# pierrepaleo/PDWT

Measured on AMD Instinct MI355X. Metric: Mpixels/s fwd+inv DWT (4096² db4 L3), higher is better.
Workload: dtype f32; 1 GPU; 4096x4096 float32, db4, 3 levels, separable DWT fwd+inv (BASELINE.json configs[1]); levels=3, parallelism=batch-split x1 (no data-path collective)

## Files before the change

### pdwt_amd/csrc/casc_dev.hpp

```cpp
#pragma once
#include "common.hpp"

#ifndef PDWT_CASC_DIAG
#define PDWT_CASC_DIAG 0
#endif
#define CASC_DIAG_ST(row) ((PDWT_CASC_DIAG & 1) ? ((row) & 31) : (row))
#define CASC_DIAG_LD(row) ((PDWT_CASC_DIAG & 2) ? ((row) & 31) : (row))

namespace pdwt {

template <int HLEN>
struct CascGeom {
    static constexpr int C = HLEN / 2 - 1;
    static constexpr int NB1 = C > 0 ? (C + 3) / 4 : 0;
    static constexpr int NB2 = C > 0 ? (C + 1) / 2 : 0;
    static constexpr int NBT = NB1 + NB2;
    static constexpr int WIN1 = 4 * (2 * NB1 + 1);
    static constexpr int WIN2 = 2 * (2 * NB2 + 1);
    static constexpr int MAXVL = 64 - 2 * NBT;
};

struct CascMap {
    int cpx;
    int strips;
    int gy;
    int flags;
    const void* tbl;
};
__host__ __device__ inline int casc_chunk_start(int g, int strip, int units, int gy, int strips, int cpx, int d)
{
    if (g >= gy) return units;
    int b = (int)(((long long)g * units) / gy);
    if (d != 0) {
        int bal = 0;
        for (int q = 0; q < g; q++) bal += (((q * strips + strip) / cpx) & 1) ? -1 : 1;
        b += d * bal;
    }
    return b;
}

struct CascBands {
    float *H1, *V1, *D1, *A2, *H2, *V2, *D2;
};
struct CascBatchF {
    const float* in;
    CascBands b;
};

template <int HLEN>
struct CascInvGeom {
    static constexpr int H2 = HLEN / 2;
    static constexpr int C = H2 / 2;
    static constexpr int SHIFT = (H2 & 1) ? 0 : 1;
    static constexpr int NB1 = C > 0 ? (C + 1) / 2 : 0;
    static constexpr int NB2 = C;
    static constexpr int NBT = NB1 + NB2;
    static constexpr int WIN1 = 2 * (2 * NB1 + 1);
    static constexpr int WIN2 = 2 * NB2 + 1;
    static constexpr int MAXVL = 64 - 2 * NBT;
    static constexpr int BASE = (C - SHIFT) & 1;
    static constexpr int VM_SB = H2 * (4 + 2 * (3 + 2));
};
struct CascInvBands {
    const float *A2, *H2, *V2, *D2, *H1, *V1, *D1;
};
struct CascInv3B {
    const float *A3, *H3, *V3, *D3;
};
struct CascBatchI {
    CascInvBands b;
    CascInv3B b3;
    float* out;
};


constexpr size_t kCascTraceOff = 1u << 20;
#ifdef PDWT_CASC_TRACE
#define CASC_TRACE_DECL unsigned long long casc_tr_[8] = {0, 0, 0, 0, 0, 0, 0, 0}
#define CASC_TRACE(i) casc_tr_[i] = wall_clock64()
#define CASC_TRACE_STORE(trash, wave_id, aux)                                                             \
    do {                                                                                                   \
        if ((threadIdx.x & 63) == 0) {                                                                     \
            unsigned long long* p_ = reinterpret_cast<unsigned long long*>((trash) + kCascTraceOff) + (size_t)(wave_id) * 8; \
            for (int i_ = 0; i_ < 7; i_++) p_[i_] = casc_tr_[i_];                                          \
            p_[7] = (unsigned long long)(aux);                                                             \
        }                                                                                                  \
    } while (0)
#else
#define CASC_TRACE_DECL
#define CASC_TRACE(i)
#define CASC_TRACE_STORE(trash, wave_id, aux)
#endif

int inv2d_casc3_f32(const float* A2, const float* H2, const float* V2, const float* D2, const float* H1, const float* V1, const float* D1,
                    const float* A3, const float* H3, const float* V3, const float* D3, float* out, float* trash, int nr, int nc, int hlen,
                    const Taps2<float>& f, const CascBatchI* d_tbl = nullptr, int nimg = 1);

int inv2d_cascw_f32(const float* A2, const float* H2, const float* V2, const float* D2, const float* H1, const float* V1, const float* D1,
                    const float* A3, const float* H3, const float* V3, const float* D3, float* out, float* trash, int nr, int nc, int hlen,
                    const Taps2<float>& f);

}
```

### pdwt_amd/csrc/common.hpp

```cpp
#pragma once
#include <atomic>
#include <hip/hip_runtime.h>
#include <hip/hip_ext.h>
#include <stddef.h>
#include <stdint.h>

#include "../../include/pdwt_hip.h"

namespace pdwt {

void set_last_error(hipError_t e, const char* what, const char* file, int line);

#define PDWT_HIP_TRY(expr)                                              \
    do {                                                                \
        hipError_t _e = (expr);                                         \
        if (_e != hipSuccess) {                                         \
            ::pdwt::set_last_error(_e, #expr, __FILE__, __LINE__);      \
            return PDWT_EHIP;                                           \
        }                                                               \
    } while (0)

hipStream_t stream();

enum KernelId {
    K_FWD2D_FUSED = 0,
    K_INV2D_FUSED,
    K_ANA_ROWS,
    K_ANA_COLS,
    K_SYN_COLS,
    K_SYN_ROWS,
    K_SWT_ANA_ROWS,
    K_SWT_ANA_COLS,
    K_SWT_SYN_COLS,
    K_SWT_SYN_ROWS,
    K_HAAR2D_FWD,
    K_HAAR2D_INV,
    K_HAAR1D_FWD,
    K_HAAR1D_INV,
    K_SOFT_THRESH,
    K_ABS_SUM,
    K_ABS_SUM_FINAL,
    K_FWD2D_CASC,
    K_INV2D_CASC,
    K_FWD2D_STREAM,
    K_INV2D_STREAM,
    K_FWD2D_SMALL,
    K_INV2D_SMALL,
    K_FWD2D_F64,
    K_INV2D_F64,
    K_THRESH_SUM,
    K_COUNT
};

struct KTimer {
    int id;
    hipEvent_t e0 = nullptr, e1 = nullptr;
    bool ext = false;
    explicit KTimer(int kernel_id, bool attach_to_launch = false);
    ~KTimer();
};
#define PDWT_LAUNCH_KT(kt, kernel, grid, block, lds, ...)                                                                  \
    do {                                                                                                                   \
        if ((kt).e0 && (kt).e1) hipExtLaunchKernelGGL(kernel, grid, block, lds, pdwt::stream(), (kt).e0, (kt).e1, 0, __VA_ARGS__); \
        else hipLaunchKernelGGL(kernel, grid, block, lds, pdwt::stream(), __VA_ARGS__);                                    \
    } while (0)

template <auto Kernel>
inline int lds_opt_in()
{
    static std::atomic<unsigned long long> done{0};
    int dev = 0;
    PDWT_HIP_TRY(hipGetDevice(&dev));
    const unsigned long long bit = 1ull << (dev & 63);
    if (!(done.load(std::memory_order_relaxed) & bit)) {
        PDWT_HIP_TRY(hipFuncSetAttribute((const void*)Kernel, hipFuncAttributeMaxDynamicSharedMemorySize, 160 * 1024));
        done.fetch_or(bit, std::memory_order_relaxed);
    }
    return PDWT_OK;
}

int lds_opt_in_ptr(const void* kernel);

unsigned long long* clock_probe_slot(int slot);
inline int clock_probe_size_class(int rows) { int c = 0; while ((rows << c) < 16384 && c < 7) c++; return c; }
constexpr int kClockProbeAllBlocks = 16384;
unsigned long long* clock_probe_all(int* all);
__device__ __forceinline__ void clock_probe_stamp(unsigned long long* probe, int second, int all = 0)
{
    if (probe && (all || (blockIdx.x == 0 && blockIdx.y == 0))) {
        unsigned long long* const p = probe + (all ? 4 * (size_t)blockIdx.x : (size_t)0);
        const unsigned long long c = clock64(), t = wall_clock64();
        if (threadIdx.x == 0) {
            p[2 * second] = c;
            p[2 * second + 1] = t;
        }
    }
}

enum KnobId {
    KN_FORCE_TWOPASS = 0,
    KN_TILED_COLS,
    KN_CASC,
    KN_CASC_WAVES,
    KN_CASC_NV,
    KN_CASC_MIN,
    KN_CASC_IWAVES,
    KN_CASC_IPFD,
    KN_CASC_WG,
    KN_CASC_IWG,
    KN_CASC_L3,
    KN_CASC_SPEC,
    KN_CASC_XCDW,
    KN_DWT1D_LDS_KB,
    KN_STREAM,
    KN_STREAM_R,
    KN_STREAM_WAVES,
    KN_STREAM_NARROW,
    KN_SMALL,
    KN_ROWS_TR,
    KN_RING_R,
    KN_RING_WAVES,
    KN_SWTF,
    KN_SWTF_M,
    KN_SWTF_MI,
    KN_SWTF_XCD,
    KN_SWTF_ALT,
    KN_SWTF_PERM,
    KN_SWTF_F64,
    KN_F64_LDS,
    KN_F64_LDS_MIN,
    KN_F64_LDS_WGS,
    KN_F64_LDS_MINGROUPS,
    KN_F64_LDS_SKEW,
    KN_NORM2SQ_REF1D,
    KN_NORM_IN_THRESHOLD,
    KN_SELFCHECK,
    KN_DWT1D_F64,
    KN_SWTF_LONG,
    KN_F64_TAIL,
    KN_EXP0,
    KN_EXP1,
    KN_EXP2,
    KN_EXP3,
    KN_NONSEP_TILED,
    KN_F64_LAT,
    KN_F64_LAT_MIN,
    KN_DWT1D_NT_MB,
    KN_COUNT
};
int knob(KnobId id);
bool counted_waits_ok();
void stat_casc_spec(int inverse);
int knob_set(const char* name, int value);
int knob_get(const char* name, int* value);

__host__ __device__ inline int div2(int n) { return (n + 1) >> 1; }
inline int idiv_up(int a, int b) { return (a + b - 1) / b; }

__device__ __forceinline__ int wrap_ext(int s, int n)
{
    const int np = n + (n & 1);
    if ((unsigned)s >= (unsigned)np) {
        s %= np;
        if (s < 0) s += np;
    }
    return (s == n) ? n - 1 : s;
}
__device__ __forceinline__ int wrap_per(int s, int n)
{
    if ((unsigned)s >= (unsigned)n) {
        s %= n;
        if (s < 0) s += n;
    }
    return s;
}

template <typename T>
struct Taps2 {
    T a[PDWT_MAX_FILTER_WIDTH];
    T b[PDWT_MAX_FILTER_WIDTH];
};

template <typename T> struct FiltersOf;
template <> struct FiltersOf<float> { using type = pdwt_filters_f32; };
template <> struct FiltersOf<double> { using type = pdwt_filters_f64; };

template <typename T>
inline Taps2<T> taps_fwd(const typename FiltersOf<T>::type* f)
{
    Taps2<T> t;
    for (int i = 0; i < PDWT_MAX_FILTER_WIDTH; i++) { t.a[i] = f->L[i]; t.b[i] = f->H[i]; }
    return t;
}
template <typename T>
inline Taps2<T> taps_inv(const typename FiltersOf<T>::type* f, T scale = T(1))
{
    Taps2<T> t;
    for (int i = 0; i < PDWT_MAX_FILTER_WIDTH; i++) { t.a[i] = f->IL[i] * scale; t.b[i] = f->IH[i] * scale; }
    return t;
}

template <typename T> __device__ __forceinline__ T fma_t(T a, T b, T c);
template <> __device__ __forceinline__ float fma_t<float>(float a, float b, float c) { return __builtin_fmaf(a, b, c); }
template <> __device__ __forceinline__ double fma_t<double>(double a, double b, double c) { return __builtin_fma(a, b, c); }

struct BandGeom {
    int nbands;
    int Nr[3 * 32 + 1], Nc[3 * 32 + 1];
    size_t alloc_elems[3 * 32 + 1];
};
int band_geometry(const pdwt_info& w, BandGeom* g);

}
```

### pdwt_amd/csrc/dwt.hip

```cpp
#include <stdlib.h>
#include <string.h>

#include "common.hpp"
#include "cols_ring.hpp"
#include "rows_tr.hpp"
#include "dwt1d_fused.hpp"
#include <new>
#include <vector>

#include "dwt_lds.hpp"
#include "dwt_lat.hpp"
#include "dwt_stream.hpp"
#include "dwt_casc.hpp"
#include "casc_dev.hpp"

namespace pdwt {

constexpr int kThreads = 256;

template <typename T, int HLEN, int TX, int TY>
__global__ __launch_bounds__(kThreads) void k_fwd2d_fused(const T* __restrict__ in, T* __restrict__ cA, T* __restrict__ cH,
                                                           T* __restrict__ cV, T* __restrict__ cD, int Nr, int Nc, int hlen_rt,
                                                           Taps2<T> f)
{
    extern __shared__ __attribute__((aligned(16))) unsigned char smem[];
    const int hlen = HLEN > 0 ? HLEN : hlen_rt;
    const int c = (hlen & 1) ? hlen / 2 : hlen / 2 - 1;
    const int RIN = 2 * TY + hlen - 2;
    const int CIN = 2 * TX + hlen - 2;
    const int CINP = CIN | 1;
    T* s_in = reinterpret_cast<T*>(smem);
    T* s_lo = s_in + RIN * CINP;
    T* s_hi = s_lo + RIN * TX;

    const int Nr2 = div2(Nr), Nc2 = div2(Nc);
    const int x0 = blockIdx.x * TX, y0 = blockIdx.y * TY;
    const int xb = 2 * x0 - c, yb = 2 * y0 - c;
    const int tx = threadIdx.x & 63, ty = threadIdx.x >> 6;

    const bool interior = (xb >= 0) && (xb + CIN <= Nc) && (yb >= 0) && (yb + RIN <= Nr);
    if (interior) {
        for (int r = ty; r < RIN; r += 4) {
            const T* row = in + (size_t)(yb + r) * Nc + xb;
            for (int cc = tx; cc < CIN; cc += 64) s_in[r * CINP + cc] = row[cc];
        }
    } else {
        for (int r = ty; r < RIN; r += 4) {
            const T* row = in + (size_t)wrap_ext(yb + r, Nr) * Nc;
            for (int cc = tx; cc < CIN; cc += 64) s_in[r * CINP + cc] = row[wrap_ext(xb + cc, Nc)];
        }
    }
    __syncthreads();

    for (int r = ty; r < RIN; r += 4) {
        const T* p = s_in + r * CINP + 2 * tx;
        T lo = 0, hi = 0;
#pragma unroll
        for (int j = 0; j < hlen; j++) {
            const T v = p[j];
            lo = fma_t(v, f.a[hlen - 1 - j], lo);
            hi = fma_t(v, f.b[hlen - 1 - j], hi);
        }
        s_lo[r * TX + tx] = lo;
        s_hi[r * TX + tx] = hi;
    }
    __syncthreads();

    const int gx = x0 + tx;
    for (int y = ty; y < TY; y += 4) {
        T a = 0, h = 0, v = 0, d = 0;
        const T* pl = s_lo + (2 * y) * TX + tx;
        const T* ph = s_hi + (2 * y) * TX + tx;
#pragma unroll
        for (int j = 0; j < hlen; j++) {
            const T l = pl[j * TX], g = ph[j * TX];
            const T fl = f.a[hlen - 1 - j], fh = f.b[hlen - 1 - j];
            a = fma_t(l, fl, a);
            h = fma_t(l, fh, h);
            v = fma_t(g, fl, v);
            d = fma_t(g, fh, d);
        }
        const int gy = y0 + y;
        if (gy < Nr2 && gx < Nc2) {
            const size_t o = (size_t)gy * Nc2 + gx;
            cA[o] = a;
            cH[o] = h;
            cV[o] = v;
            cD[o] = d;
        }
    }
}

template <typename T, int HLEN, int TX, int TY>
__global__ __launch_bounds__(kThreads) void k_inv2d_fused(const T* __restrict__ cA, const T* __restrict__ cH, const T* __restrict__ cV,
                                                           const T* __restrict__ cD, T* __restrict__ out, int Nri, int Nci, int Nro,
                                                           int Nco, int hlen_rt, Taps2<T> f)
{
    extern __shared__ __attribute__((aligned(16))) unsigned char smem[];
    const int hlen = HLEN > 0 ? HLEN : hlen_rt;
    const int h2 = hlen / 2;
    const int c = h2 / 2;
    const int shift = (h2 & 1) ? 0 : 1;
    const int RC = TY + h2;
    const int CC = TX + h2;
    const int CCP = CC | 1;
    T* s_A = reinterpret_cast<T*>(smem);
    T* s_H = s_A + RC * CCP;
    T* s_V = s_H + RC * CCP;
    T* s_D = s_V + RC * CCP;
    T* s_t1 = s_D + RC * CCP;
    T* s_t2 = s_t1 + 2 * TY * CCP;

    const int x0 = blockIdx.x * TX, y0 = blockIdx.y * TY;
    const int xb = x0 - c, yb = y0 - c;
    const int tx = threadIdx.x & 63, ty = threadIdx.x >> 6;

    const bool interior = (xb >= 0) && (xb + CC <= Nci) && (yb >= 0) && (yb + RC <= Nri);
    for (int r = ty; r < RC; r += 4) {
        const size_t ro = (size_t)(interior ? yb + r : wrap_per(yb + r, Nri)) * Nci;
        for (int cc = tx; cc < CC; cc += 64) {
            const size_t o = ro + (interior ? xb + cc : wrap_per(xb + cc, Nci));
            const int s = r * CCP + cc;
            s_A[s] = cA[o];
            s_H[s] = cH[o];
            s_V[s] = cV[o];
            s_D[s] = cD[o];
        }
    }
    __syncthreads();

    for (int gyl = ty; gyl < 2 * TY; gyl += 4) {
        const int gp = gyl + shift;
        const int pl = gp >> 1, off = 1 - (gp & 1);
        for (int cc = tx; cc < CC; cc += 64) {
            T sa = 0, sh = 0, sv = 0, sd = 0;
            const int base = pl * CCP + cc;
#pragma unroll
            for (int j = 0; j < h2; j++) {
                const int k = hlen - 1 - (2 * j + off);
                const T fl = f.a[k], fh = f.b[k];
                const int s = base + j * CCP;
                sa = fma_t(s_A[s], fl, sa);
                sh = fma_t(s_H[s], fh, sh);
                sv = fma_t(s_V[s], fl, sv);
                sd = fma_t(s_D[s], fh, sd);
            }
            s_t1[gyl * CCP + cc] = sa + sh;
            s_t2[gyl * CCP + cc] = sv + sd;
        }
    }
    __syncthreads();

    for (int gyl = ty; gyl < 2 * TY; gyl += 4) {
        const int gy = 2 * y0 + gyl;
        if (gy >= Nro) break;
        for (int u = tx; u < TX; u += 64) {
            T res[2];
#pragma unroll
            for (int e = 0; e < 2; e++) {
                const int gp = 2 * u + e + shift;
                const int pl = gp >> 1, off = 1 - ((e + shift) & 1);
                T s1 = 0, s2 = 0;
                const int base = gyl * CCP + pl;
#pragma unroll
                for (int j = 0; j < h2; j++) {
                    const int k = hlen - 1 - (2 * j + off);
                    s1 = fma_t(s_t1[base + j], f.a[k], s1);
                    s2 = fma_t(s_t2[base + j], f.b[k], s2);
                }
                res[e] = s1 + s2;
            }
            const int gx = 2 * x0 + 2 * u;
            if (gx < Nco) out[(size_t)gy * Nco + gx] = res[0];
            if (gx + 1 < Nco) out[(size_t)gy * Nco + gx + 1] = res[1];
        }
    }
}

template <typename T, int HLEN, int TXO>
__global__ __launch_bounds__(kThreads) void k_ana_rows(const T* __restrict__ in, T* __restrict__ lo, T* __restrict__ hi, int Nr, int Nc,
                                                        int hlen_rt, Taps2<T> f)
{
    extern __shared__ __attribute__((aligned(16))) unsigned char smem[];
    const int hlen = HLEN > 0 ? HLEN : hlen_rt;
    const int c = (hlen & 1) ? hlen / 2 : hlen / 2 - 1;
    const int CIN = 2 * TXO + hlen - 2;
    const int CINP = CIN | 1;
    const int lane = threadIdx.x & 63, w = threadIdx.x >> 6;
    T* s = reinterpret_cast<T*>(smem) + w * CINP;
    const int Nc2 = div2(Nc);
    const int x0 = blockIdx.x * TXO;
    const int xb = 2 * x0 - c;
    const int row = blockIdx.y * 4 + w;
    if (row < Nr) {
        const T* src = in + (size_t)row * Nc;
        if (xb >= 0 && xb + CIN <= Nc) {
            for (int cc = lane; cc < CIN; cc += 64) s[cc] = src[xb + cc];
        } else {
            for (int cc = lane; cc < CIN; cc += 64) s[cc] = src[wrap_ext(xb + cc, Nc)];
        }
    }
    __syncthreads();
    if (row >= Nr) return;
    for (int i = lane; i < TXO; i += 64) {
        const int gx = x0 + i;
        if (gx >= Nc2) break;
        const T* p = s + 2 * i;
        T l = 0, h = 0;
#pragma unroll
        for (int j = 0; j < hlen; j++) {
            const T v = p[j];
            l = fma_t(v, f.a[hlen - 1 - j], l);
            h = fma_t(v, f.b[hlen - 1 - j], h);
        }
        lo[(size_t)row * Nc2 + gx] = l;
        hi[(size_t)row * Nc2 + gx] = h;
    }
}

template <typename T, int HLEN, int TYO>
__global__ __launch_bounds__(kThreads) void k_ana_cols(const T* __restrict__ t1, const T* __restrict__ t2, T* __restrict__ cA,
                                                        T* __restrict__ cH, T* __restrict__ cV, T* __restrict__ cD, int Nr, int Ncw,
                                                        int hlen_rt, Taps2<T> f)
{
    extern __shared__ __attribute__((aligned(16))) unsigned char smem[];
    const int hlen = HLEN > 0 ? HLEN : hlen_rt;
    const int c = (hlen & 1) ? hlen / 2 : hlen / 2 - 1;
    const int RIN = 2 * TYO + hlen - 2;
    T* s1 = reinterpret_cast<T*>(smem);
    T* s2 = s1 + RIN * 64;
    const int tx = threadIdx.x & 63, ty = threadIdx.x >> 6;
    const int Nr2 = div2(Nr);
    const int gx = blockIdx.x * 64 + tx;
    const int y0 = blockIdx.y * TYO;
    const int yb = 2 * y0 - c;
    if (gx < Ncw) {
        for (int r = ty; r < RIN; r += 4) {
            const size_t o = (size_t)wrap_ext(yb + r, Nr) * Ncw + gx;
            s1[r * 64 + tx] = t1[o];
            s2[r * 64 + tx] = t2[o];
        }
    }
    __syncthreads();
    if (gx >= Ncw) return;
    for (int y = ty; y < TYO; y += 4) {
        const int gy = y0 + y;
        if (gy >= Nr2) break;
        T a = 0, h = 0, v = 0, d = 0;
        const T* p1 = s1 + (2 * y) * 64 + tx;
        const T* p2 = s2 + (2 * y) * 64 + tx;
#pragma unroll
        for (int j = 0; j < hlen; j++) {
            const T l = p1[j * 64], g = p2[j * 64];
            const T fl = f.a[hlen - 1 - j], fh = f.b[hlen - 1 - j];
            a = fma_t(l, fl, a);
            h = fma_t(l, fh, h);
            v = fma_t(g, fl, v);
            d = fma_t(g, fh, d);
        }
        const size_t o = (size_t)gy * Ncw + gx;
        cA[o] = a;
        cH[o] = h;
        cV[o] = v;
        cD[o] = d;
    }
}

template <typename T, int HLEN, int TYC>
__global__ __launch_bounds__(kThreads) void k_syn_cols(const T* __restrict__ cA, const T* __restrict__ cH, const T* __restrict__ cV,
                                                        const T* __restrict__ cD, T* __restrict__ t1, T* __restrict__ t2, int Nri,
                                                        int Nc, int Nro, int hlen_rt, Taps2<T> f)
{
    extern __shared__ __attribute__((aligned(16))) unsigned char smem[];
    const int hlen = HLEN > 0 ? HLEN : hlen_rt;
    const int h2 = hlen / 2;
    const int c = h2 / 2;
    const int shift = (h2 & 1) ? 0 : 1;
    const int RC = TYC + h2;
    T* s_A = reinterpret_cast<T*>(smem);
    T* s_H = s_A + RC * 64;
    T* s_V = s_H + RC * 64;
    T* s_D = s_V + RC * 64;
    const int tx = threadIdx.x & 63, ty = threadIdx.x >> 6;
    const int gx = blockIdx.x * 64 + tx;
    const int y0 = blockIdx.y * TYC;
    const int yb = y0 - c;
    if (gx < Nc) {
        for (int r = ty; r < RC; r += 4) {
            const size_t o = (size_t)wrap_per(yb + r, Nri) * Nc + gx;
            const int s = r * 64 + tx;
            s_A[s] = cA[o];
            s_H[s] = cH[o];
            s_V[s] = cV[o];
            s_D[s] = cD[o];
        }
    }
    __syncthreads();
    if (gx >= Nc) return;
    for (int gyl = ty; gyl < 2 * TYC; gyl += 4) {
        const int gy = 2 * y0 + gyl;
        if (gy >= Nro) break;
        const int gp = gyl + shift;
        const int pl = gp >> 1, off = 1 - (gp & 1);
        T sa = 0, sh = 0, sv = 0, sd = 0;
        const int base = pl * 64 + tx;
#pragma unroll
        for (int j = 0; j < h2; j++) {
            const int k = hlen - 1 - (2 * j + off);
            const T fl = f.a[k], fh = f.b[k];
            const int s = base + j * 64;
            sa = fma_t(s_A[s], fl, sa);
            sh = fma_t(s_H[s], fh, sh);
            sv = fma_t(s_V[s], fl, sv);
            sd = fma_t(s_D[s], fh, sd);
        }
        t1[(size_t)gy * Nc + gx] = sa + sh;
        t2[(size_t)gy * Nc + gx] = sv + sd;
    }
}

template <typename T, int HLEN, int TXC>
__global__ __launch_bounds__(kThreads) void k_syn_rows(const T* __restrict__ a, const T* __restrict__ d, T* __restrict__ out, int Nr,
                                                        int Nci, int Nco, int hlen_rt, Taps2<T> f)
{
    extern __shared__ __attribute__((aligned(16))) unsigned char smem[];
    const int hlen = HLEN > 0 ? HLEN : hlen_rt;
    const int h2 = hlen / 2;
    const int c = h2 / 2;
    const int shift = (h2 & 1) ? 0 : 1;
    const int CC = TXC + h2;
    const int lane = threadIdx.x & 63, w = threadIdx.x >> 6;
    T* sa = reinterpret_cast<T*>(smem) + w * 2 * CC;
    T* sd = sa + CC;
    const int x0 = blockIdx.x * TXC;
    const int xb = x0 - c;
    const int row = blockIdx.y * 4 + w;
    if (row < Nr) {
        const T* pa = a + (size_t)row * Nci;
        const T* pd = d + (size_t)row * Nci;
        for (int cc = lane; cc < CC; cc += 64) {
            const int sx = wrap_per(xb + cc, Nci);
            sa[cc] = pa[sx];
            sd[cc] = pd[sx];
        }
    }
    __syncthreads();
    if (row >= Nr) return;
    for (int u = lane; u < TXC; u += 64) {
        const int gx = 2 * x0 + 2 * u;
        if (gx >= Nco) break;
        T res[2];
#pragma unroll
        for (int e = 0; e < 2; e++) {
            const int gp = 2 * u + e + shift;
            const int pl = gp >> 1, off = 1 - ((e + shift) & 1);
            T s1 = 0, s2 = 0;
#pragma unroll
            for (int j = 0; j < h2; j++) {
                const int k = hlen - 1 - (2 * j + off);
                s1 = fma_t(sa[pl + j], f.a[k], s1);
                s2 = fma_t(sd[pl + j], f.b[k], s2);
            }
            res[e] = s1 + s2;
        }
        out[(size_t)row * Nco + gx] = res[0];
        if (gx + 1 < Nco) out[(size_t)row * Nco + gx + 1] = res[1];
    }
}

template <typename K>
static int set_lds(K kernel, size_t bytes)
{
    if (bytes > 64 * 1024) return lds_opt_in_ptr((const void*)kernel);
    return PDWT_OK;
}

static bool force_twopass() { return knob(KN_FORCE_TWOPASS) == 1; }
static bool tiled_cols_forced() { return knob(KN_TILED_COLS) == 1; }

constexpr int FTX = 64, FTY = 16;
constexpr size_t kFusedLdsBudget = 64 * 1024;

template <typename T>
static size_t fwd_fused_lds(int hlen)
{
    const int RIN = 2 * FTY + hlen - 2, CINP = (2 * FTX + hlen - 2) | 1;
    return ((size_t)RIN * CINP + 2 * (size_t)RIN * FTX) * sizeof(T);
}
template <typename T>
static size_t inv_fused_lds(int hlen)
{
    const int h2 = hlen / 2, RC = FTY + h2, CCP = (FTX + h2) | 1;
    return (4 * (size_t)RC * CCP + 2 * (size_t)(2 * FTY) * CCP) * sizeof(T);
}

#define PDWT_CHECK_LAUNCH() PDWT_HIP_TRY(hipGetLastError())

#define PDWT_TILED_HLENS(X) X(4) X(6) X(8) X(10) X(12) X(14) X(16) X(18) X(20) X(24) X(30) X(40)

template <typename T>
static int launch_ana_rows(const T* in, T* lo, T* hi, int Nr, int Nc, int hlen, const Taps2<T>& f)
{
    if constexpr (sizeof(T) == 8) {
        const int rc = ana_rows_tr_f64(in, lo, hi, Nr, Nc, hlen, f);
        if (rc <= 0) return rc;
    }
    constexpr int TXO = 256;
    const size_t lds = 4 * (size_t)((2 * TXO + hlen - 2) | 1) * sizeof(T);
    dim3 grid(idiv_up(div2(Nc), TXO), idiv_up(Nr, 4));
    void (*k)(const T*, T*, T*, int, int, int, Taps2<T>);
    switch (hlen) {
#define X(H) case H: k = k_ana_rows<T, H, TXO>; break;
        PDWT_TILED_HLENS(X)
#undef X
        default: k = k_ana_rows<T, 0, TXO>; break;
    }
    KTimer kt(K_ANA_ROWS);
    hipLaunchKernelGGL(k, grid, dim3(kThreads), lds, stream(), in, lo, hi, Nr, Nc, hlen, f);
    PDWT_CHECK_LAUNCH();
    return PDWT_OK;
}

template <typename T>
static int launch_syn_rows(const T* a, const T* d, T* out, int Nr, int Nci, int Nco, int hlen, const Taps2<T>& f)
{
    if constexpr (sizeof(T) == 8) {
        const int rc = syn_rows_tr_f64(a, d, out, Nr, Nci, Nco, hlen, f);
        if (rc <= 0) return rc;
    }
    constexpr int TXC = 128;
    const size_t lds = 4 * 2 * (size_t)(TXC + hlen / 2) * sizeof(T);
    dim3 grid(idiv_up(Nci, TXC), idiv_up(Nr, 4));
    void (*k)(const T*, const T*, T*, int, int, int, int, Taps2<T>);
    switch (hlen) {
#define X(H) case H: k = k_syn_rows<T, H, TXC>; break;
        PDWT_TILED_HLENS(X)
#undef X
        default: k = k_syn_rows<T, 0, TXC>; break;
    }
    KTimer kt(K_SYN_ROWS);
    hipLaunchKernelGGL(k, grid, dim3(kThreads), lds, stream(), a, d, out, Nr, Nci, Nco, hlen, f);
    PDWT_CHECK_LAUNCH();
    return PDWT_OK;
}

template <typename T>
static int launch_ana_cols(const T* t1, const T* t2, T* cA, T* cH, T* cV, T* cD, int Nr, int Ncw, int hlen, const Taps2<T>& f)
{
    if (!tiled_cols_forced()) {
        KTimer kt(K_ANA_COLS);
        const int rc = ana_cols_ring<T>(t1, cA, cH, Nr, Ncw, hlen, f, t2, cV, cD);
        if (rc <= 0) return rc;
    }
    constexpr int TYO = 16;
    const size_t lds = 2 * (size_t)(2 * TYO + hlen - 2) * 64 * sizeof(T);
    void (*k)(const T*, const T*, T*, T*, T*, T*, int, int, int, Taps2<T>);
    switch (hlen) {
#define X(H) case H: k = k_ana_cols<T, H, TYO>; break;
        PDWT_TILED_HLENS(X)
#undef X
        default: k = k_ana_cols<T, 0, TYO>; break;
    }
    if (set_lds(k, lds) != PDWT_OK) return PDWT_EHIP;
    dim3 grid(idiv_up(Ncw, 64), idiv_up(div2(Nr), TYO));
    KTimer kt(K_ANA_COLS);
    hipLaunchKernelGGL(k, grid, dim3(kThreads), lds, stream(), t1, t2, cA, cH, cV, cD, Nr, Ncw, hlen, f);
    PDWT_CHECK_LAUNCH();
    return PDWT_OK;
}

template <typename T>
static int launch_syn_cols(const T* cA, const T* cH, const T* cV, const T* cD, T* t1, T* t2, int Nri, int Nc, int Nro, int hlen,
                           const Taps2<T>& f)
{
    if (!tiled_cols_forced()) {
        KTimer kt(K_SYN_COLS);
        const int rc = syn_cols_ring<T>(cA, cH, t1, Nri, Nc, Nro, hlen, f, cV, cD, t2);
        if (rc <= 0) return rc;
    }
    constexpr int TYC = 16;
    const size_t lds = 4 * (size_t)(TYC + hlen / 2) * 64 * sizeof(T);
    void (*k)(const T*, const T*, const T*, const T*, T*, T*, int, int, int, int, Taps2<T>);
    switch (hlen) {
#define X(H) case H: k = k_syn_cols<T, H, TYC>; break;
        PDWT_TILED_HLENS(X)
#undef X
        default: k = k_syn_cols<T, 0, TYC>; break;
    }
    if (set_lds(k, lds) != PDWT_OK) return PDWT_EHIP;
    dim3 grid(idiv_up(Nc, 64), idiv_up(Nri, TYC));
    KTimer kt(K_SYN_COLS);
    hipLaunchKernelGGL(k, grid, dim3(kThreads), lds, stream(), cA, cH, cV, cD, t1, t2, Nri, Nc, Nro, hlen, f);
    PDWT_CHECK_LAUNCH();
    return PDWT_OK;
}

template <typename T>
static int level_fwd2d(const T* in, T* cA, T* cH, T* cV, T* cD, T* t1, T* t2, size_t trash_floats, int nr, int nc, int hlen, const Taps2<T>& f,
                       T* taps_dev)
{
    if constexpr (sizeof(T) == 8) {
        if (!force_twopass()) {
            int rc = fwd2d_f64_lat(in, cA, cH, cV, cD, nr, nc, hlen, f);
            if (rc <= 0) return rc;
            rc = fwd2d_f64_lds(in, cA, cH, cV, cD, taps_dev, nr, nc, hlen, f);
            if (rc <= 0) return rc;
        }
    }
    if constexpr (sizeof(T) == 4) {
        if (!force_twopass()) {
            int rc = fwd2d_stream_f32(in, cA, cH, cV, cD, (float*)t1, trash_floats, nr, nc, hlen, f);
            if (rc <= 0) return rc;
            rc = fwd2d_f32_lds(in, cA, cH, cV, cD, nr, nc, hlen, f);
            if (rc <= 0) return rc;
        }
    }
    const size_t lds = fwd_fused_lds<T>(hlen);
    if (lds <= kFusedLdsBudget && !force_twopass()) {
        dim3 grid(idiv_up(div2(nc), FTX), idiv_up(div2(nr), FTY));
        void (*k)(const T*, T*, T*, T*, T*, int, int, int, Taps2<T>);
        switch (hlen) {
#define X(H) case H: k = k_fwd2d_fused<T, H, FTX, FTY>; break;
            PDWT_TILED_HLENS(X)
#undef X
            default: k = k_fwd2d_fused<T, 0, FTX, FTY>; break;
        }
        KTimer kt(K_FWD2D_FUSED);
        hipLaunchKernelGGL(k, grid, dim3(kThreads), lds, stream(), in, cA, cH, cV, cD, nr, nc, hlen, f);
        PDWT_CHECK_LAUNCH();
        return PDWT_OK;
    }
    int rc = launch_ana_rows(in, t1, t2, nr, nc, hlen, f);
    if (rc != PDWT_OK) return rc;
    return launch_ana_cols(t1, t2, cA, cH, cV, cD, nr, div2(nc), hlen, f);
}

template <typename T>
static int level_inv2d(const T* cA, const T* cH, const T* cV, const T* cD, T* out, T* t1, T* t2, int nri, int nci, int nro, int nco,
                       int hlen, const Taps2<T>& f, T* taps_dev)
{
    if constexpr (sizeof(T) == 8) {
        if (!force_twopass()) {
            int rc = inv2d_f64_lat(cA, cH, cV, cD, out, nri, nci, nro, nco, hlen, f);
            if (rc <= 0) return rc;
            rc = inv2d_f64_lds(cA, cH, cV, cD, out, taps_dev, nri, nci, nro, nco, hlen, f);
            if (rc <= 0) return rc;
        }
    }
    if constexpr (sizeof(T) == 4) {
        if (!force_twopass()) {
            int rc = inv2d_stream_f32(cA, cH, cV, cD, out, nri, nci, nro, nco, hlen, f);
            if (rc <= 0) return rc;
            rc = inv2d_f32_lds(cA, cH, cV, cD, out, nri, nci, nro, nco, hlen, f);
            if (rc <= 0) return rc;
        }
    }
    const size_t lds = inv_fused_lds<T>(hlen);
    if (lds <= kFusedLdsBudget && !force_twopass()) {
        dim3 grid(idiv_up(nci, FTX), idiv_up(nri, FTY));
        void (*k)(const T*, const T*, const T*, const T*, T*, int, int, int, int, int, Taps2<T>);
        switch (hlen) {
#define X(H) case H: k = k_inv2d_fused<T, H, FTX, FTY>; break;
            PDWT_TILED_HLENS(X)
#undef X
            default: k = k_inv2d_fused<T, 0, FTX, FTY>; break;
        }
        KTimer kt(K_INV2D_FUSED);
        hipLaunchKernelGGL(k, grid, dim3(kThreads), lds, stream(), cA, cH, cV, cD, out, nri, nci, nro, nco, hlen, f);
        PDWT_CHECK_LAUNCH();
        return PDWT_OK;
    }
    int rc = launch_syn_cols(cA, cH, cV, cD, t1, t2, nri, nci, nro, hlen, f);
    if (rc != PDWT_OK) return rc;
    return launch_syn_rows(t1, t2, out, nro, nci, nco, hlen, f);
}

template <typename T>
struct Scratch {
    T *t1, *t2, *ping[2];
    size_t trash_floats;
    bool t1_is_trash;
    Scratch(T* tmp, int Nr, int Nc, int ndims)
    {
        t1_is_trash = (ndims == 2) && ((size_t)Nr * div2(Nc) * sizeof(T) >= kStreamTrashFloats * sizeof(float)) && Nr >= 32;
        auto up = [](size_t n) { return (n + 63) & ~(size_t)63; };
        const size_t half = up((size_t)Nr * div2(Nc));
        trash_floats = (ndims == 2) ? 2 * half * sizeof(T) / sizeof(float) : 0;
        const size_t quarter = up((size_t)(ndims == 2 ? div2(Nr) : Nr) * div2(Nc));
        t1 = tmp;
        t2 = t1 + half;
        if (ndims == 2) {
            ping[0] = t2 + half;
            ping[1] = ping[0] + quarter;
        } else {
            ping[0] = tmp;
            ping[1] = tmp + quarter;
        }
    }
};

static int check_args(const void* img, const void* coeffs, const void* tmp, const pdwt_info& w, int ndims, bool need_filters, const void* f,
                      int fhlen)
{
    if (!img || !coeffs || !tmp) return PDWT_EINVAL;
    if (w.Nr < 1 || w.Nc < 1 || w.nlevels < 1 || w.nlevels > 32) return PDWT_EINVAL;
    if (w.ndims != ndims) return PDWT_EINVAL;
    if (need_filters) {
        if (!f) return PDWT_EINVAL;
        if (w.hlen < 2 || w.hlen > PDWT_MAX_FILTER_WIDTH || fhlen != w.hlen) return PDWT_EINVAL;
    }
    return PDWT_OK;
}

template <typename T>
static int forward_separable(T* d_image, T** c, T* d_tmp, pdwt_info w, const typename FiltersOf<T>::type* filt)
{
    int rc = check_args(d_image, c, d_tmp, w, 2, true, filt, filt ? filt->hlen : 0);
    if (rc != PDWT_OK) return rc;
    const Taps2<T> f = taps_fwd<T>(filt);
    Scratch<T> s(d_tmp, w.Nr, w.Nc, 2);
    const T* in = d_image;
    int nr = w.Nr, nc = w.Nc;
    int pp = 0;
    for (int lev = 0; lev < w.nlevels; lev++) {
        if constexpr (sizeof(T) == 4) {
            if (lev + 1 < w.nlevels && !force_twopass()) {
                T* a2 = (lev + 2 == w.nlevels) ? c[0] : s.ping[pp];
                float* trash = s.t1_is_trash ? (float*)s.t1 : nullptr;
                rc = fwd2d_casc_f32(in, c[3 * lev + 1], c[3 * lev + 2], c[3 * lev + 3], a2, c[3 * lev + 4], c[3 * lev + 5], c[3 * lev + 6],
                                    trash, nr, nc, w.hlen, f);
                if (rc < 0) return rc;
                if (rc == PDWT_OK) {
                    in = a2;
                    pp ^= 1;
                    nr = div2(div2(nr));
                    nc = div2(div2(nc));
                    lev++;
                    continue;
                }
            }
        }
        T* aout = (lev == w.nlevels - 1) ? c[0] : s.ping[pp];
        rc = level_fwd2d(in, aout, c[3 * lev + 1], c[3 * lev + 2], c[3 * lev + 3], s.t1, s.t2, s.trash_floats, nr, nc, w.hlen, f,
                         d_tmp + pdwt_tmp_elems(w) - 256);
        if (rc != PDWT_OK) return rc;
        in = aout;
        pp ^= 1;
        nr = div2(nr);
        nc = div2(nc);
    }
    return PDWT_OK;
}

template <typename T>
static int inverse_separable(T* d_image, T** c, T* d_tmp, pdwt_info w, const typename FiltersOf<T>::type* filt)
{
    int rc = check_args(d_image, c, d_tmp, w, 2, true, filt, filt ? filt->hlen : 0);
    if (rc != PDWT_OK) return rc;
    const Taps2<T> f = taps_inv<T>(filt);
    Scratch<T> s(d_tmp, w.Nr, w.Nc, 2);
    int tNr[34], tNc[34];
    tNr[0] = w.Nr;
    tNc[0] = w.Nc;
    for (int i = 1; i <= w.nlevels; i++) {
        tNr[i] = div2(tNr[i - 1]);
        tNc[i] = div2(tNc[i - 1]);
    }
    const T* a = c[0];
    int top = w.nlevels - 1;
    int pp = (a == s.ping[0]) ? 1 : 0;
    for (int i = top; i >= 0; i--) {
        if constexpr (sizeof(T) == 4) {
            float* trash = s.t1_is_trash ? (float*)s.t1 : nullptr;
            if (i >= 2 && !(i & 1) && !force_twopass()) {
                T* out = (i == 2) ? d_image : s.ping[pp];
                rc = inv2d_cascw_f32(nullptr, c[3 * i - 2], c[3 * i - 1], c[3 * i], c[3 * i - 5], c[3 * i - 4], c[3 * i - 3], a, c[3 * i + 1],
                                     c[3 * i + 2], c[3 * i + 3], out, trash, tNr[i - 2], tNc[i - 2], w.hlen, f);
                if (rc < 0) return rc;
                if (rc == PDWT_OK) {
                    a = out;
                    pp ^= 1;
                    i -= 2;
                    continue;
                }
            }
            if ((i & 1) && !force_twopass()) {
                T* out = (i == 1) ? d_image : s.ping[pp];
                rc = inv2d_cascw_f32(a, c[3 * i + 1], c[3 * i + 2], c[3 * i + 3], c[3 * i - 2], c[3 * i - 1], c[3 * i], nullptr, nullptr, nullptr,
                                     nullptr, out, trash, tNr[i - 1], tNc[i - 1], w.hlen, f);
                if (rc < 0) return rc;
                if (rc == PDWT_OK) {
                    a = out;
                    pp ^= 1;
                    i--;
                    continue;
                }
                rc = inv2d_casc_f32(a, c[3 * i + 1], c[3 * i + 2], c[3 * i + 3], c[3 * i - 2], c[3 * i - 1], c[3 * i], out, trash, tNr[i - 1],
                                    tNc[i - 1], w.hlen, f);
                if (rc < 0) return rc;
                if (rc == PDWT_OK) {
                    a = out;
                    pp ^= 1;
                    i--;
                    continue;
                }
            }
        }
        T* out = (i == 0) ? d_image : s.ping[pp];
        rc = level_inv2d(a, c[3 * i + 1], c[3 * i + 2], c[3 * i + 3], out, s.t1, s.t2, tNr[i + 1], tNc[i + 1], tNr[i], tNc[i], w.hlen, f,
                         d_tmp + pdwt_tmp_elems(w) - 256);
        if (rc != PDWT_OK) return rc;
        a = out;
        pp ^= 1;
    }
    return PDWT_OK;
}

template <typename T>
static int forward_separable_1d(T* d_image, T** c, T* d_tmp, pdwt_info w, const typename FiltersOf<T>::type* filt)
{
    int rc = check_args(d_image, c, d_tmp, w, 1, true, filt, filt ? filt->hlen : 0);
    if (rc != PDWT_OK) return rc;
    const Taps2<T> f = taps_fwd<T>(filt);
    if (!force_twopass()) {
        rc = fwd1d_fused<T>(d_image, c, w, f);
        if (rc <= 0) return rc;
    }
    Scratch<T> s(d_tmp, w.Nr, w.Nc, 1);
    const T* in = d_image;
    int nc = w.Nc;
    for (int lev = 0; lev < w.nlevels; lev++) {
        T* aout = (lev == w.nlevels - 1) ? c[0] : s.ping[lev & 1];
        rc = launch_ana_rows(in, aout, c[lev + 1], w.Nr, nc, w.hlen, f);
        if (rc != PDWT_OK) return rc;
        in = aout;
        nc = div2(nc);
    }
    return PDWT_OK;
}

template <typename T>
static int inverse_separable_1d(T* d_image, T** c, T* d_tmp, pdwt_info w, const typename FiltersOf<T>::type* filt)
{
    int rc = check_args(d_image, c, d_tmp, w, 1, true, filt, filt ? filt->hlen : 0);
    if (rc != PDWT_OK) return rc;
    const Taps2<T> f = taps_inv<T>(filt);
    if (!force_twopass()) {
        rc = inv1d_fused<T>(d_image, c, w, f);
        if (rc <= 0) return rc;
    }
    Scratch<T> s(d_tmp, w.Nr, w.Nc, 1);
    int tNc[34];
    tNc[0] = w.Nc;
    for (int i = 1; i <= w.nlevels; i++) tNc[i] = div2(tNc[i - 1]);
    const T* a = c[0];
    for (int i = w.nlevels - 1; i >= 0; i--) {
        T* out = (i == 0) ? d_image : s.ping[i & 1];
        rc = launch_syn_rows(a, (const T*)c[i + 1], out, w.Nr, tNc[i + 1], tNc[i], w.hlen, f);
        if (rc != PDWT_OK) return rc;
        a = out;
    }
    return PDWT_OK;
}


static inline bool b2_al16(const void* p) { return ((uintptr_t)p & 15) == 0; }
template <typename T> void* haar_batch_create(int nimg, T* const* d_images, T** const* d_coeffs, T* const* d_tmps, pdwt_info w);
template <typename T> int haar_batch_forward(void* batch);
template <typename T> int haar_batch_inverse(void* batch);
template <typename T> void haar_batch_destroy(void* batch);
void* swt_batch_create_f32(int nimg, float* const* d_images, float** const* d_coeffs, float* const* d_tmps, pdwt_info w);
int swt_batch_forward_f32(void* batch, const pdwt_filters_f32* filt);
int swt_batch_inverse_f32(void* batch, const pdwt_filters_f32* filt);
void swt_batch_destroy_f32(void* batch);
struct BatchHaar {
    int kind, dev, elem;
    void* hb;
};
static void* batch_swt_create(int nimg, float* const* d_images, float** const* d_coeffs, float* const* d_tmps, pdwt_info w)
{
    BatchHaar* B = new (std::nothrow) BatchHaar();
    if (!B) return nullptr;
    B->kind = 3;
    B->elem = 4;
    B->hb = (hipGetDevice(&B->dev) == hipSuccess) ? swt_batch_create_f32(nimg, d_images, d_coeffs, d_tmps, w) : nullptr;
    if (!B->hb) {
        delete B;
        return nullptr;
    }
    return B;
}
template <typename T>
static void* batch_haar_create(int nimg, T* const* d_images, T** const* d_coeffs, T* const* d_tmps, pdwt_info w)
{
    BatchHaar* B = new (std::nothrow) BatchHaar();
    if (!B) return nullptr;
    B->kind = 2;
    B->elem = (int)sizeof(T);
    B->hb = (hipGetDevice(&B->dev) == hipSuccess) ? haar_batch_create<T>(nimg, d_images, d_coeffs, d_tmps, w) : nullptr;
    if (!B->hb) {
        delete B;
        return nullptr;
    }
    return B;
}
struct Batch2D {
    int kind;
    int nimg, dev;
    pdwt_info w;
    size_t trash_floats;
    int lev_nr[33], lev_nc[33];
    StreamBatchF* d_fwd;
    StreamBatchI* d_inv;
    CascBatchF* d_cf;
    CascBatchI* d_ci;
    CascBatchF cf0;
    CascBatchI ci0;
    float* trash0;
};

static Batch2D* batch2d_create(int nimg, float* const* d_images, float** const* d_coeffs, float* const* d_tmps, pdwt_info w, int hlen)
{
    if (nimg < 1 || nimg > 65535 || !d_images || !d_coeffs || !d_tmps || w.ndims != 2 || w.do_swt || w.nlevels < 1 || w.nlevels > 32) return nullptr;
    if (force_twopass()) return nullptr;
    int nr = w.Nr, nc = w.Nc;
    for (int lev = 0; lev < w.nlevels; lev++) {
        if (!fwd2d_stream_takes(nr, nc, hlen) || !inv2d_stream_takes(nr / 2, nc / 2, hlen)) return nullptr;
        nr /= 2;
        nc /= 2;
    }
    Scratch<float> probe(d_tmps[0], w.Nr, w.Nc, 2);
    if (probe.trash_floats < 1024) return nullptr;
    Batch2D* B = new (std::nothrow) Batch2D();
    if (!B) return nullptr;
    B->kind = 0;
    B->nimg = nimg;
    B->w = w;
    B->trash_floats = probe.trash_floats;
    B->d_fwd = nullptr;
    B->d_inv = nullptr;
    B->d_cf = nullptr;
    B->d_ci = nullptr;
    B->trash0 = nullptr;
    if (hipGetDevice(&B->dev) != hipSuccess) {
        delete B;
        return nullptr;
    }
    const int L = w.nlevels;
    std::vector<StreamBatchF> hf((size_t)L * nimg);
    std::vector<StreamBatchI> hi((size_t)L * nimg);
    for (int b = 0; b < nimg; b++) {
        float* const* c = d_coeffs[b];
        Scratch<float> s(d_tmps[b], w.Nr, w.Nc, 2);
        if (!d_images[b] || !c || !d_tmps[b] || !b2_al16(d_images[b])) {
            delete B;
            return nullptr;
        }
        const float* in = d_images[b];
        int pp = 0;
        for (int lev = 0; lev < L; lev++) {
            float* aout = (lev == L - 1) ? c[0] : s.ping[pp];
            hf[(size_t)lev * nimg + b] = StreamBatchF{in, aout, c[3 * lev + 1], c[3 * lev + 2], c[3 * lev + 3], (float*)s.t1};
            if (!b2_al16(aout) || !b2_al16(c[3 * lev + 1]) || !b2_al16(c[3 * lev + 2]) || !b2_al16(c[3 * lev + 3])) {
                delete B;
                return nullptr;
            }
            in = aout;
            pp ^= 1;
        }
        const float* a = c[0];
        pp = 0;
        for (int i = L - 1; i >= 0; i--) {
            float* out = (i == 0) ? d_images[b] : s.ping[pp];
            hi[(size_t)i * nimg + b] = StreamBatchI{a, c[3 * i + 1], c[3 * i + 2], c[3 * i + 3], out};
            a = out;
            pp ^= 1;
        }
    }
    nr = w.Nr;
    nc = w.Nc;
    for (int lev = 0; lev <= L; lev++) {
        B->lev_nr[lev] = nr;
        B->lev_nc[lev] = nc;
        nr /= 2;
        nc /= 2;
    }
    const size_t bf = hf.size() * sizeof(StreamBatchF), bi = hi.size() * sizeof(StreamBatchI);
    B->d_fwd = (StreamBatchF*)pdwt_malloc(bf);
    B->d_inv = (StreamBatchI*)pdwt_malloc(bi);
    bool ok = B->d_fwd && B->d_inv && pdwt_memcpy_h2d(B->d_fwd, hf.data(), bf) == PDWT_OK && pdwt_memcpy_h2d(B->d_inv, hi.data(), bi) == PDWT_OK;
    if (ok && L >= 2) {
        std::vector<CascBatchF> hcf((size_t)nimg);
        std::vector<CascBatchI> hci((size_t)nimg);
        for (int b = 0; b < nimg; b++) {
            float* const* c = d_coeffs[b];
            hcf[b] = CascBatchF{d_images[b], CascBands{c[1], c[2], c[3], hf[(size_t)1 * nimg + b].cA, c[4], c[5], c[6]}};
            hci[b].b = CascInvBands{L == 2 ? hi[(size_t)1 * nimg + b].cA : nullptr, c[4], c[5], c[6], c[1], c[2], c[3]};
            hci[b].b3 = (L >= 3) ? CascInv3B{hi[(size_t)2 * nimg + b].cA, c[7], c[8], c[9]} : CascInv3B{nullptr, nullptr, nullptr, nullptr};
            hci[b].out = d_images[b];
        }
        B->cf0 = hcf[0];
        B->ci0 = hci[0];
        Scratch<float> s0(d_tmps[0], w.Nr, w.Nc, 2);
        B->trash0 = s0.t1_is_trash ? (float*)s0.t1 : nullptr;
        const size_t cf = hcf.size() * sizeof(CascBatchF), ci = hci.size() * sizeof(CascBatchI);
        B->d_cf = (CascBatchF*)pdwt_malloc(cf);
        B->d_ci = (CascBatchI*)pdwt_malloc(ci);
        ok = B->d_cf && B->d_ci && pdwt_memcpy_h2d(B->d_cf, hcf.data(), cf) == PDWT_OK && pdwt_memcpy_h2d(B->d_ci, hci.data(), ci) == PDWT_OK;
    }
    if (!ok) {
        pdwt_free(B->d_fwd);
        pdwt_free(B->d_inv);
        pdwt_free(B->d_cf);
        pdwt_free(B->d_ci);
        delete B;
        return nullptr;
    }
    return B;
}

struct Batch2DDev {
    int prev = -1;
    bool switched = false;
    explicit Batch2DDev(int dev)
    {
        if (hipGetDevice(&prev) == hipSuccess && prev != dev) switched = (hipSetDevice(dev) == hipSuccess);
    }
    ~Batch2DDev()
    {
        if (switched) (void)hipSetDevice(prev);
    }
};

static int batch2d_forward(Batch2D* B, const pdwt_filters_f32* filt)
{
    if (!B || !filt || filt->hlen != B->w.hlen) return PDWT_EINVAL;
    Batch2DDev on_dev(B->dev);
    const Taps2<float> f = taps_fwd<float>(filt);
    int lev0 = 0;
    if (B->d_cf && B->trash0) {
        const CascBands& b = B->cf0.b;
        const int rc = fwd2d_casc_f32(B->cf0.in, b.H1, b.V1, b.D1, b.A2, b.H2, b.V2, b.D2, B->trash0, B->lev_nr[0], B->lev_nc[0], B->w.hlen, f,
                                      B->d_cf, B->nimg);
        if (rc < 0) return rc;
        if (rc == PDWT_OK) lev0 = 2;
    }
    for (int lev = lev0; lev < B->w.nlevels; lev++) {
        const int rc = fwd2d_stream_batch_f32(B->d_fwd + (size_t)lev * B->nimg, B->nimg, B->trash_floats, B->lev_nr[lev], B->lev_nc[lev], B->w.hlen, f);
        if (rc != PDWT_OK) return rc < 0 ? rc : PDWT_EINVAL;
    }
    return PDWT_OK;
}

static int batch2d_inverse(Batch2D* B, const pdwt_filters_f32* filt)
{
    if (!B || !filt || filt->hlen != B->w.hlen) return PDWT_EINVAL;
    Batch2DDev on_dev(B->dev);
    const Taps2<float> f = taps_inv<float>(filt);
    const int L = B->w.nlevels;
    const int ncasc = (L >= 3) ? 3 : 2;
    bool casc = B->d_ci && B->trash0 && L >= 2 && knob(KN_CASC) == 1 && knob(KN_CASC_IWG) != 1 && knob(KN_CASC_L3) == 1 && stream_enabled() &&
                !((long long)knob(KN_CASC_MIN) > (long long)B->lev_nr[0] * B->lev_nc[0]);
    int next = L - 1;
    for (; next >= (casc ? ncasc : 0); next--) {
        const int rc = inv2d_stream_batch_f32(B->d_inv + (size_t)next * B->nimg, B->nimg, B->lev_nr[next + 1], B->lev_nc[next + 1], B->w.hlen, f);
        if (rc != PDWT_OK) return rc < 0 ? rc : PDWT_EINVAL;
    }
    if (casc) {
        const CascInvBands& b = B->ci0.b;
        const CascInv3B& b3 = B->ci0.b3;
        const int rc = inv2d_casc3_f32(b.A2, b.H2, b.V2, b.D2, b.H1, b.V1, b.D1, b3.A3, b3.H3, b3.V3, b3.D3, B->ci0.out, B->trash0, B->lev_nr[0],
                                       B->lev_nc[0], B->w.hlen, f, B->d_ci, B->nimg);
        if (rc < 0) return rc;
        if (rc == PDWT_OK) return PDWT_OK;
    }
    for (; next >= 0; next--) {
        const int rc = inv2d_stream_batch_f32(B->d_inv + (size_t)next * B->nimg, B->nimg, B->lev_nr[next + 1], B->lev_nc[next + 1], B->w.hlen, f);
        if (rc != PDWT_OK) return rc < 0 ? rc : PDWT_EINVAL;
    }
    return PDWT_OK;
}

struct Batch2D64 {
    int kind;
    int nimg, dev;
    pdwt_info w;
    int lev_nr[34], lev_nc[34];
    unsigned long long* d_fwd;
    unsigned long long* d_inv;
};

static Batch2D64* batch2d_create_f64(int nimg, double* const* d_images, double** const* d_coeffs, double* const* d_tmps, pdwt_info w)
{
    if (nimg < 1 || nimg > 65535 || !d_images || !d_coeffs || !d_tmps || w.ndims != 2 || w.do_swt || w.nlevels < 1 || w.nlevels > 32) return nullptr;
    if (force_twopass() || w.hlen < 2 || w.hlen > 40 || (w.hlen & 1) || knob(KN_F64_LDS) < 1) return nullptr;
    Batch2D64* B = new (std::nothrow) Batch2D64();
    if (!B) return nullptr;
    B->kind = 1;
    B->nimg = nimg;
    B->w = w;
    B->d_fwd = B->d_inv = nullptr;
    if (hipGetDevice(&B->dev) != hipSuccess) {
        delete B;
        return nullptr;
    }
    const int L = w.nlevels;
    int nr = w.Nr, nc = w.Nc;
    for (int lev = 0; lev <= L; lev++) {
        B->lev_nr[lev] = nr;
        B->lev_nc[lev] = nc;
        const int hp = ((w.hlen + 7) / 8) * 8;
        if (lev < L && (nr < 16 || nr < hp || nc < hp || div2(nr) < hp || div2(nc) < 2)) {
            delete B;
            return nullptr;
        }
        nr = div2(nr);
        nc = div2(nc);
    }
    std::vector<unsigned long long> hf((size_t)L * nimg * 5), hi((size_t)L * nimg * 5);
    for (int b = 0; b < nimg; b++) {
        double* const* c = d_coeffs[b];
        if (!d_images[b] || !c || !d_tmps[b]) {
            delete B;
            return nullptr;
        }
        Scratch<double> sc(d_tmps[b], w.Nr, w.Nc, 2);
        const double* in = d_images[b];
        int pp = 0;
        for (int lev = 0; lev < L; lev++) {
            double* aout = (lev == L - 1) ? c[0] : sc.ping[pp];
            unsigned long long* e = &hf[((size_t)lev * nimg + b) * 5];
            e[0] = (unsigned long long)(uintptr_t)in;
            e[1] = (unsigned long long)(uintptr_t)aout;
            e[2] = (unsigned long long)(uintptr_t)c[3 * lev + 1];
            e[3] = (unsigned long long)(uintptr_t)c[3 * lev + 2];
            e[4] = (unsigned long long)(uintptr_t)c[3 * lev + 3];
            if (!aout || !c[3 * lev + 1] || !c[3 * lev + 2] || !c[3 * lev + 3]) {
                delete B;
                return nullptr;
            }
            in = aout;
            pp ^= 1;
        }
        const double* a = c[0];
        pp = 0;
        for (int i = L - 1; i >= 0; i--) {
            double* out = (i == 0) ? d_images[b] : sc.ping[pp];
            unsigned long long* e = &hi[((size_t)i * nimg + b) * 5];
            e[0] = (unsigned long long)(uintptr_t)a;
            e[1] = (unsigned long long)(uintptr_t)c[3 * i + 1];
            e[2] = (unsigned long long)(uintptr_t)c[3 * i + 2];
            e[3] = (unsigned long long)(uintptr_t)c[3 * i + 3];
            e[4] = (unsigned long long)(uintptr_t)out;
            a = out;
            pp ^= 1;
        }
    }
    const size_t bytes = hf.size() * sizeof(unsigned long long);
    B->d_fwd = (unsigned long long*)pdwt_malloc(bytes);
    B->d_inv = (unsigned long long*)pdwt_malloc(bytes);
    if (!B->d_fwd || !B->d_inv || pdwt_memcpy_h2d(B->d_fwd, hf.data(), bytes) != PDWT_OK || pdwt_memcpy_h2d(B->d_inv, hi.data(), bytes) != PDWT_OK) {
        pdwt_free(B->d_fwd);
        pdwt_free(B->d_inv);
        delete B;
        return nullptr;
    }
    return B;
}

static int batch2d_forward_f64(Batch2D64* B, const pdwt_filters_f64* filt)
{
    if (!B || !filt || filt->hlen != B->w.hlen) return PDWT_EINVAL;
    Batch2DDev on_dev(B->dev);
    const Taps2<double> f = taps_fwd<double>(filt);
    for (int lev = 0; lev < B->w.nlevels; lev++) {
        const int rc = fwd2d_f64_lds_batch(B->d_fwd + (size_t)lev * B->nimg * 5, B->nimg, B->lev_nr[lev], B->lev_nc[lev], B->w.hlen, f);
        if (rc != PDWT_OK) return rc < 0 ? rc : PDWT_EINVAL;
    }
    return PDWT_OK;
}
static int batch2d_inverse_f64(Batch2D64* B, const pdwt_filters_f64* filt)
{
    if (!B || !filt || filt->hlen != B->w.hlen) return PDWT_EINVAL;
    Batch2DDev on_dev(B->dev);
    const Taps2<double> f = taps_inv<double>(filt);
    for (int i = B->w.nlevels - 1; i >= 0; i--) {
        const int rc = inv2d_f64_lds_batch(B->d_inv + (size_t)i * B->nimg * 5, B->nimg, B->lev_nr[i + 1], B->lev_nc[i + 1], B->lev_nr[i], B->lev_nc[i], B->w.hlen, f);
        if (rc != PDWT_OK) return rc < 0 ? rc : PDWT_EINVAL;
    }
    return PDWT_OK;
}

}

template <typename F>
static bool bank_is_haar(const F* f)
{
    if (!f || f->hlen != 2) return false;
    const double r = 0.70710678118654752440, tol = 1e-6;
    auto near = [&](double a, double b) { return a - b <= tol && b - a <= tol; };
    return near(f->L[0], r) && near(f->L[1], r) && near(f->H[0], -r) && near(f->H[1], r) && near(f->IL[0], r) && near(f->IL[1], r) && near(f->IH[0], r) && near(f->IH[1], -r);
}

using namespace pdwt;

extern "C" {
static bool batch_is_haar(const pdwt_info& w) { return w.hlen == 2 && w.ndims == 2 && !w.do_swt; }
void* pdwt_batch2d_create_f64(int nimg, double* const* d_images, double** const* d_coeffs, double* const* d_tmps, pdwt_info info)
{
    if (batch_is_haar(info)) return batch_haar_create<double>(nimg, d_images, d_coeffs, d_tmps, info);
    return batch2d_create_f64(nimg, d_images, d_coeffs, d_tmps, info);
}
static int batch_kind(const void* batch, int elem)
{
    if (!batch) return -1;
    const int k = *(const int*)batch;
    if (k == 0 || k == 3) return elem == 4 ? k : -1;
    if (k == 1) return elem == 8 ? k : -1;
    if (k == 2) return ((const BatchHaar*)batch)->elem == elem ? k : -1;
    return -1;
}
int pdwt_batch2d_forward_f64(void* batch, const pdwt_filters_f64* f)
{
    const int k = batch_kind(batch, 8);
    if (k == 2) {
        if (!bank_is_haar(f)) return PDWT_EINVAL;
        Batch2DDev on_dev(((BatchHaar*)batch)->dev);
        return haar_batch_forward<double>(((BatchHaar*)batch)->hb);
    }
    return k == 1 ? batch2d_forward_f64((Batch2D64*)batch, f) : PDWT_EINVAL;
}
int pdwt_batch2d_inverse_f64(void* batch, const pdwt_filters_f64* f)
{
    const int k = batch_kind(batch, 8);
    if (k == 2) {
        if (!bank_is_haar(f)) return PDWT_EINVAL;
        Batch2DDev on_dev(((BatchHaar*)batch)->dev);
        return haar_batch_inverse<double>(((BatchHaar*)batch)->hb);
    }
    return k == 1 ? batch2d_inverse_f64((Batch2D64*)batch, f) : PDWT_EINVAL;
}
void* pdwt_batch2d_create_f32(int nimg, float* const* d_images, float** const* d_coeffs, float* const* d_tmps, pdwt_info info)
{
    if (batch_is_haar(info)) return batch_haar_create<float>(nimg, d_images, d_coeffs, d_tmps, info);
    if (info.do_swt) return batch_swt_create(nimg, d_images, d_coeffs, d_tmps, info);
    return batch2d_create(nimg, d_images, d_coeffs, d_tmps, info, info.hlen);
}
int pdwt_batch2d_forward_f32(void* batch, const pdwt_filters_f32* f)
{
    const int k = batch_kind(batch, 4);
    if (k == 2 || k == 3) {
        if (k == 2 && !bank_is_haar(f)) return PDWT_EINVAL;
        Batch2DDev on_dev(((BatchHaar*)batch)->dev);
        return k == 2 ? haar_batch_forward<float>(((BatchHaar*)batch)->hb) : swt_batch_forward_f32(((BatchHaar*)batch)->hb, f);
    }
    return k == 0 ? batch2d_forward((Batch2D*)batch, f) : PDWT_EINVAL;
}
int pdwt_batch2d_inverse_f32(void* batch, const pdwt_filters_f32* f)
{
    const int k = batch_kind(batch, 4);
    if (k == 2 || k == 3) {
        if (k == 2 && !bank_is_haar(f)) return PDWT_EINVAL;
        Batch2DDev on_dev(((BatchHaar*)batch)->dev);
        return k == 2 ? haar_batch_inverse<float>(((BatchHaar*)batch)->hb) : swt_batch_inverse_f32(((BatchHaar*)batch)->hb, f);
    }
    return k == 0 ? batch2d_inverse((Batch2D*)batch, f) : PDWT_EINVAL;
}
void pdwt_batch2d_destroy(void* batch)
{
    if (!batch) return;
    const int k = *(const int*)batch;
    if (k == 2 || k == 3) {
        BatchHaar* H = (BatchHaar*)batch;
        if (k == 3)
            swt_batch_destroy_f32(H->hb);
        else if (H->elem == 8)
            haar_batch_destroy<double>(H->hb);
        else
            haar_batch_destroy<float>(H->hb);
        delete H;
    } else if (k == 1) {
        Batch2D64* B = (Batch2D64*)batch;
        pdwt_free(B->d_fwd);
        pdwt_free(B->d_inv);
        delete B;
    } else if (k == 0) {
        Batch2D* B = (Batch2D*)batch;
        pdwt_free(B->d_fwd);
        pdwt_free(B->d_inv);
        pdwt_free(B->d_cf);
        pdwt_free(B->d_ci);
        delete B;
    }
}
void pdwt_batch2d_destroy_f64(void* batch) { pdwt_batch2d_destroy(batch); }
int pdwt_debug_set(const char* key, int value) { return pdwt::knob_set(key, value); }
int pdwt_debug_get(const char* key, int* value) { return pdwt::knob_get(key, value); }
size_t pdwt_tmp_elems(pdwt_info w) { return 2 * (size_t)(w.Nr > 0 ? w.Nr : 0) * (size_t)(w.Nc > 0 ? w.Nc : 0) + 1024; }
int pdwt_forward_separable_f32(float* i, float** c, float* t, pdwt_info w, const pdwt_filters_f32* f) { return forward_separable<float>(i, c, t, w, f); }
int pdwt_forward_separable_f64(double* i, double** c, double* t, pdwt_info w, const pdwt_filters_f64* f) { return forward_separable<double>(i, c, t, w, f); }
int pdwt_inverse_separable_f32(float* i, float** c, float* t, pdwt_info w, const pdwt_filters_f32* f) { return inverse_separable<float>(i, c, t, w, f); }
int pdwt_inverse_separable_f64(double* i, double** c, double* t, pdwt_info w, const pdwt_filters_f64* f) { return inverse_separable<double>(i, c, t, w, f); }
int pdwt_forward_separable_1d_f32(float* i, float** c, float* t, pdwt_info w, const pdwt_filters_f32* f) { return forward_separable_1d<float>(i, c, t, w, f); }
int pdwt_forward_separable_1d_f64(double* i, double** c, double* t, pdwt_info w, const pdwt_filters_f64* f) { return forward_separable_1d<double>(i, c, t, w, f); }
int pdwt_inverse_separable_1d_f32(float* i, float** c, float* t, pdwt_info w, const pdwt_filters_f32* f) { return inverse_separable_1d<float>(i, c, t, w, f); }
int pdwt_inverse_separable_1d_f64(double* i, double** c, double* t, pdwt_info w, const pdwt_filters_f64* f) { return inverse_separable_1d<double>(i, c, t, w, f); }
}
```

### pdwt_amd/csrc/dwt_casc.hip

```cpp
#include "dwt_casc.hpp"

#include <algorithm>

#include "dwt_stream.hpp"
#include "stream_dev.hpp"
#include "casc_dev.hpp"

namespace pdwt {

constexpr int casc_fwd_stores(int p) { return 3 + 4 * (p & 1); }
template <int DIST>
constexpr int casc_fwd_after(int p)
{
    int n = casc_fwd_stores(p);
    for (int k = 1; k < DIST; k++) n += 2 + casc_fwd_stores(p + k);
    return n;
}

template <int HLEN>
constexpr int casc_fwd_region_bytes() { return (HLEN - 2) * 64 * (16 + 8); }

#define PDWT_VB_F0 " op_sel_hi:[0,1,0]"
#define PDWT_VB_N0 " op_sel_hi:[0,1,1]"
#define PDWT_VB_F1 " op_sel:[1,0,0] op_sel_hi:[1,1,0]"
#define PDWT_VB_N1 " op_sel:[1,0,0]"
template <bool WITH_VD>
__device__ __forceinline__ void col_pass8x2(v2f& ah0, v2f& ah1, v2f& vd0, v2f& vd1, v2f a0, v2f a1, v2f a2, v2f a3, v2f a4, v2f a5, v2f a6, v2f a7, v2f b0, v2f b1,
                                            v2f b2, v2f b3, v2f b4, v2f b5, v2f b6, v2f b7, v2f t0, v2f t1, v2f t2, v2f t3, v2f t4, v2f t5, v2f t6, v2f t7)
{
#define PDWT_CP_ROW(A, B, T, AC)                                                                                              \
    "v_pk_fma_f32 %0, " A ", " T ", " AC "0\n\tv_pk_fma_f32 %1, " B ", " T ", " AC "1\n\t"
    if constexpr (WITH_VD) {
        asm("v_pk_fma_f32 %0, %4, %20, 0" PDWT_VB_F0 "\n\tv_pk_fma_f32 %1, %12, %20, 0" PDWT_VB_F0 "\n\tv_pk_fma_f32 %2, %4, %20, 0" PDWT_VB_F1 "\n\tv_pk_fma_f32 %3, %12, %20, 0" PDWT_VB_F1
            "\n\tv_pk_fma_f32 %0, %5, %21, %0" PDWT_VB_N0 "\n\tv_pk_fma_f32 %1, %13, %21, %1" PDWT_VB_N0 "\n\tv_pk_fma_f32 %2, %5, %21, %2" PDWT_VB_N1 "\n\tv_pk_fma_f32 %3, %13, %21, %3" PDWT_VB_N1
            "\n\tv_pk_fma_f32 %0, %6, %22, %0" PDWT_VB_N0 "\n\tv_pk_fma_f32 %1, %14, %22, %1" PDWT_VB_N0 "\n\tv_pk_fma_f32 %2, %6, %22, %2" PDWT_VB_N1 "\n\tv_pk_fma_f32 %3, %14, %22, %3" PDWT_VB_N1
            "\n\tv_pk_fma_f32 %0, %7, %23, %0" PDWT_VB_N0 "\n\tv_pk_fma_f32 %1, %15, %23, %1" PDWT_VB_N0 "\n\tv_pk_fma_f32 %2, %7, %23, %2" PDWT_VB_N1 "\n\tv_pk_fma_f32 %3, %15, %23, %3" PDWT_VB_N1
            "\n\tv_pk_fma_f32 %0, %8, %24, %0" PDWT_VB_N0 "\n\tv_pk_fma_f32 %1, %16, %24, %1" PDWT_VB_N0 "\n\tv_pk_fma_f32 %2, %8, %24, %2" PDWT_VB_N1 "\n\tv_pk_fma_f32 %3, %16, %24, %3" PDWT_VB_N1
            "\n\tv_pk_fma_f32 %0, %9, %25, %0" PDWT_VB_N0 "\n\tv_pk_fma_f32 %1, %17, %25, %1" PDWT_VB_N0 "\n\tv_pk_fma_f32 %2, %9, %25, %2" PDWT_VB_N1 "\n\tv_pk_fma_f32 %3, %17, %25, %3" PDWT_VB_N1
            "\n\tv_pk_fma_f32 %0, %10, %26, %0" PDWT_VB_N0 "\n\tv_pk_fma_f32 %1, %18, %26, %1" PDWT_VB_N0 "\n\tv_pk_fma_f32 %2, %10, %26, %2" PDWT_VB_N1 "\n\tv_pk_fma_f32 %3, %18, %26, %3" PDWT_VB_N1
            "\n\tv_pk_fma_f32 %0, %11, %27, %0" PDWT_VB_N0 "\n\tv_pk_fma_f32 %1, %19, %27, %1" PDWT_VB_N0 "\n\tv_pk_fma_f32 %2, %11, %27, %2" PDWT_VB_N1 "\n\tv_pk_fma_f32 %3, %19, %27, %3" PDWT_VB_N1
            : "=&v"(ah0), "=&v"(ah1), "=&v"(vd0), "=&v"(vd1)
            : "v"(a0), "v"(a1), "v"(a2), "v"(a3), "v"(a4), "v"(a5), "v"(a6), "v"(a7), "v"(b0), "v"(b1), "v"(b2), "v"(b3), "v"(b4), "v"(b5), "v"(b6), "v"(b7),
              "s"(t0), "s"(t1), "s"(t2), "s"(t3), "s"(t4), "s"(t5), "s"(t6), "s"(t7));
    } else {
        asm("v_pk_fma_f32 %0, %2, %18, 0" PDWT_VB_F0 "\n\tv_pk_fma_f32 %1, %10, %18, 0" PDWT_VB_F0
            "\n\tv_pk_fma_f32 %0, %3, %19, %0" PDWT_VB_N0 "\n\tv_pk_fma_f32 %1, %11, %19, %1" PDWT_VB_N0
            "\n\tv_pk_fma_f32 %0, %4, %20, %0" PDWT_VB_N0 "\n\tv_pk_fma_f32 %1, %12, %20, %1" PDWT_VB_N0
            "\n\tv_pk_fma_f32 %0, %5, %21, %0" PDWT_VB_N0 "\n\tv_pk_fma_f32 %1, %13, %21, %1" PDWT_VB_N0
            "\n\tv_pk_fma_f32 %0, %6, %22, %0" PDWT_VB_N0 "\n\tv_pk_fma_f32 %1, %14, %22, %1" PDWT_VB_N0
            "\n\tv_pk_fma_f32 %0, %7, %23, %0" PDWT_VB_N0 "\n\tv_pk_fma_f32 %1, %15, %23, %1" PDWT_VB_N0
            "\n\tv_pk_fma_f32 %0, %8, %24, %0" PDWT_VB_N0 "\n\tv_pk_fma_f32 %1, %16, %24, %1" PDWT_VB_N0
            "\n\tv_pk_fma_f32 %0, %9, %25, %0" PDWT_VB_N0 "\n\tv_pk_fma_f32 %1, %17, %25, %1" PDWT_VB_N0
            : "=&v"(ah0), "=&v"(ah1)
            : "v"(a0), "v"(a1), "v"(a2), "v"(a3), "v"(a4), "v"(a5), "v"(a6), "v"(a7), "v"(b0), "v"(b1), "v"(b2), "v"(b3), "v"(b4), "v"(b5), "v"(b6), "v"(b7),
              "s"(t0), "s"(t1), "s"(t2), "s"(t3), "s"(t4), "s"(t5), "s"(t6), "s"(t7));
    }
#undef PDWT_CP_ROW
}
__device__ __forceinline__ void col_pass8x1(v2f& ah, v2f& vd, v2f a0, v2f a1, v2f a2, v2f a3, v2f a4, v2f a5, v2f a6, v2f a7, v2f t0, v2f t1, v2f t2, v2f t3, v2f t4,
                                            v2f t5, v2f t6, v2f t7)
{
    asm("v_pk_fma_f32 %0, %2, %10, 0" PDWT_VB_F0 "\n\tv_pk_fma_f32 %1, %2, %10, 0" PDWT_VB_F1
        "\n\tv_pk_fma_f32 %0, %3, %11, %0" PDWT_VB_N0 "\n\tv_pk_fma_f32 %1, %3, %11, %1" PDWT_VB_N1
        "\n\tv_pk_fma_f32 %0, %4, %12, %0" PDWT_VB_N0 "\n\tv_pk_fma_f32 %1, %4, %12, %1" PDWT_VB_N1
        "\n\tv_pk_fma_f32 %0, %5, %13, %0" PDWT_VB_N0 "\n\tv_pk_fma_f32 %1, %5, %13, %1" PDWT_VB_N1
        "\n\tv_pk_fma_f32 %0, %6, %14, %0" PDWT_VB_N0 "\n\tv_pk_fma_f32 %1, %6, %14, %1" PDWT_VB_N1
        "\n\tv_pk_fma_f32 %0, %7, %15, %0" PDWT_VB_N0 "\n\tv_pk_fma_f32 %1, %7, %15, %1" PDWT_VB_N1
        "\n\tv_pk_fma_f32 %0, %8, %16, %0" PDWT_VB_N0 "\n\tv_pk_fma_f32 %1, %8, %16, %1" PDWT_VB_N1
        "\n\tv_pk_fma_f32 %0, %9, %17, %0" PDWT_VB_N0 "\n\tv_pk_fma_f32 %1, %9, %17, %1" PDWT_VB_N1
        : "=&v"(ah), "=&v"(vd)
        : "v"(a0), "v"(a1), "v"(a2), "v"(a3), "v"(a4), "v"(a5), "v"(a6), "v"(a7), "s"(t0), "s"(t1), "s"(t2), "s"(t3), "s"(t4), "s"(t5), "s"(t6), "s"(t7));
}

template <int HLEN, int R2, bool LV, int DIST>
struct CascSpec {
    static constexpr int NA = 2 * R2, NA1 = NA + HLEN - 2, NL1 = NA - HLEN / 2 + 1;
    static constexpr int LIM = LV ? NA1 : NL1;
    static constexpr int stores_at(int q) { return ((q < NA) ? 3 : 0) + (((q & 1) && q >= HLEN - 1) ? 4 : 0); }
    static constexpr int loads_at(int q) { return (q < LIM && q + DIST < LIM) ? 2 : 0; }
    static constexpr int wait_cnt(int n)
    {
        const int m = n - DIST;
        int c = stores_at(m);
        for (int k = 1; k < DIST; k++) c += loads_at(m + k) + stores_at(m + k);
        return c;
    }
};

template <int HLEN, int NV, int W, bool SPEC = false>
__global__ __launch_bounds__(W == 1 ? 256 : 64 * W) void k_fwd2d_casc(const float* in, CascBands b, int Nr, int Nc, int VL,
                                                                       float* __restrict__ trash, CascMap cm, TapsLH f)
{
    using G = CascGeom<HLEN>;
    constexpr int C = G::C, NB1 = G::NB1, NB2 = G::NB2, NBT = G::NBT, WIN1 = G::WIN1, WIN2 = G::WIN2;
    extern __shared__ __attribute__((aligned(16))) unsigned char lds_raw[];
    CASC_TRACE_DECL;
    CASC_TRACE(0);
    if constexpr (W > 1) {
        if (cm.tbl) {
            static_assert(sizeof(CascBatchF) == 8 * sizeof(void*), "eight pointers per image");
            typedef const unsigned long long __attribute__((address_space(4))) * tbl_t;
            const tbl_t q = (tbl_t)(const unsigned long long*)cm.tbl + 8 * (size_t)blockIdx.y;
            in = (const float*)q[0];
            b = CascBands{(float*)q[1], (float*)q[2], (float*)q[3], (float*)q[4], (float*)q[5], (float*)q[6], (float*)q[7]};
        }
    }
    const int lane = threadIdx.x & 63;
    const int Nc2 = Nc >> 1, Nr2 = Nr >> 1, Nr4 = Nr >> 2, Nc4 = Nc >> 2;
    const int kw = __builtin_amdgcn_readfirstlane(threadIdx.x >> 6);
    int j0, rows2, strip;
    bool last;
    if constexpr (W == 1) {
        const int xcd = blockIdx.x & 7;
        const int wi = (blockIdx.x >> 3) * 4 + kw;
        if (wi >= cm.cpx * cm.strips) return;
        const int cy = xcd * cm.cpx + wi / cm.strips;
        strip = wi % cm.strips;
        const int nchunks = 8 * cm.cpx;
        j0 = (int)(((long long)cy * Nr4) / nchunks);
        rows2 = (int)(((long long)(cy + 1) * Nr4) / nchunks) - j0;
        if (rows2 <= 0) return;
        last = true;
    } else {
        const int xcd = blockIdx.x & 7, slot = blockIdx.x >> 3;
        const int wg = xcd * cm.cpx + slot;
        if (slot >= cm.cpx || wg >= cm.gy * cm.strips) return;
        const int gy = wg / cm.strips;
        strip = wg % cm.strips;
        const int J0 = casc_chunk_start(gy, strip, Nr4, cm.gy, cm.strips, cm.cpx, cm.flags);
        const int R = casc_chunk_start(gy + 1, strip, Nr4, cm.gy, cm.strips, cm.cpx, cm.flags) - J0;
        const int E = min((3 * (HLEN - 2) + 3) / 4, R / W - 1);
        const int base = (R + E) / W, rem = (R + E) % W;
        const int start = kw * base + min(kw, rem);
        rows2 = (kw < W - 1) ? base + (kw < rem ? 1 : 0) : R - start;
        j0 = J0 + start;
        last = (kw == W - 1);
    }
    const int xs = strip * VL * 4;
    const int x = xs + 4 * (lane - NBT);
    const bool valid = (lane >= NBT) && (lane < NBT + VL) && (x < Nc);
    const int xo = wrapi(x, Nc);
    const int yb = 4 * j0 - 3 * C;
    const int NA = 2 * rows2;
    const int NA1 = NA + HLEN - 2;
    const int NL1 = NA - HLEN / 2 + 1;
    const int rlast = last ? 2 * NA1 + HLEN - 3 : 2 * NA - 1;

    v2f ring[HLEN][2];
    v2f ring2[HLEN];
#pragma unroll
    for (int k = 0; k < HLEN; k++) ring2[k] = v2f{0.f, 0.f};

    const float* const lbase = in + xo;
    auto rowptr = [&](int r) { return lbase + (size_t)wrap1(yb + r, Nr) * Nc; };
    const unsigned xoff = (unsigned)xo * 4u;

    constexpr int REG = casc_fwd_region_bytes<HLEN>();
    unsigned char* const lds_rd = lds_raw + (size_t)(W > 1 ? kw : 0) * REG;
    unsigned char* const lds_wr = lds_raw + (size_t)(W > 1 && kw > 0 ? kw - 1 : 0) * REG;
    auto lds_ring = [&](unsigned char* reg, int r) { return reinterpret_cast<v4f*>(reg + ((size_t)r * 64 + lane) * 16); };
    auto lds_ring2 = [&](unsigned char* reg, int r) { return reinterpret_cast<v2f*>(reg + (size_t)(HLEN - 2) * 64 * 16 + ((size_t)r * 64 + lane) * 8); };
    auto row_pass1 = [&](const v4f& v, v2f (&lh)[2]) {
        float w[WIN1];
#pragma unroll
        for (int q = 0; q < 4; q++) w[NB1 * 4 + q] = v[q];
#pragma unroll
        for (int k = 0; k < NB1; k++) {
            const int dl = (NB1 - 1 - k) * 4, sl = (NB1 - k) * 4, dr = (NB1 + 1 + k) * 4, sr = (NB1 + k) * 4;
#pragma unroll
            for (int q = 0; q < 4; q++) {
                w[dl + q] = dpp_shr1(w[sl + q]);
                w[dr + q] = dpp_shl1(w[sr + q]);
            }
        }
#pragma unroll
        for (int p = 0; p < 2; p++) {
            v2f acc = {0.f, 0.f};
#pragma unroll
            for (int j = 0; j < HLEN; j++) acc = pk_fma(splat(w[NB1 * 4 - C + 2 * p + j]), f.t[HLEN - 1 - j], acc);
            lh[p] = acc;
        }
    };
    auto row_pass2 = [&](float a0, float a1, v2f& lh) {
        float w[WIN2];
        w[NB2 * 2] = a0;
        w[NB2 * 2 + 1] = a1;
#pragma unroll
        for (int k = 0; k < NB2; k++) {
            const int dl = (NB2 - 1 - k) * 2, sl = (NB2 - k) * 2, dr = (NB2 + 1 + k) * 2, sr = (NB2 + k) * 2;
#pragma unroll
            for (int q = 0; q < 2; q++) {
                w[dl + q] = dpp_shr1(w[sl + q]);
                w[dr + q] = dpp_shl1(w[sr + q]);
            }
        }
        v2f acc = {0.f, 0.f};
#pragma unroll
        for (int j = 0; j < HLEN; j++) acc = pk_fma(splat(w[NB2 * 2 - C + j]), f.t[HLEN - 1 - j], acc);
        lh = acc;
    };

    constexpr int DIST = NV / 2;
    static_assert(casc_fwd_after<DIST>(1) <= 63, "vmcnt is a 6-bit counter");
    v4f v[NV];
    {
        v4f pv[HLEN > 2 ? HLEN - 2 : 1];
#pragma unroll
        for (int r = 0; r < HLEN - 2; r++) pv[r] = *reinterpret_cast<const v4f*>(rowptr(r));
#pragma unroll
        for (int u = 0; u < NV; u++) v[u] = *reinterpret_cast<const v4f*>(rowptr(min(HLEN - 2 + u, rlast)));
        static_for<HLEN - 2>([&](auto Rr) {
            constexpr int r = decltype(Rr)::value;
            row_pass1(pv[r], ring[r]);
        });
    }
    if constexpr (W > 1) {
        if (kw > 0) {
#pragma unroll
            for (int r = 0; r < HLEN - 2; r++) *lds_ring(lds_wr, r) = v4f{ring[r][0].x, ring[r][0].y, ring[r][1].x, ring[r][1].y};
        }
    }

    const unsigned off1 = (unsigned)(valid ? x >> 1 : 0) * 4u, off2 = (unsigned)(valid ? x >> 2 : 0) * 4u;
    const lanemask_t vmask = __ballot(valid);
    const int lim1 = ((W == 1) || last) ? 0x7fffffff : NL1;
    const int lim2 = ((W == 1) || last) ? 0x7fffffff : NA;
    int lr = HLEN - 2 + NV;
    int lgr = wrap1(yb + min(lr, rlast), Nr);
    const size_t strideB = (size_t)Nc * 4;
    const char* const inB = reinterpret_cast<const char*>(in);
    const char* lp = inB + (size_t)lgr * strideB;
    const char* lplast = lp;
    auto next_rows = [&](const char*& p0, const char*& p1) {
        int lrq = lr;
        asm("" : "+s"(lrq));
        if (lrq < rlast) {
            p0 = lp;
            if (lgr + 2 < Nr) {
                p1 = lp + strideB;
                lp = p1 + strideB;
                lgr += 2;
            } else {
                p1 = (lgr + 1 == Nr) ? inB : lp + strideB;
                lgr = lgr + 2 - Nr;
                lp = inB + (size_t)lgr * strideB;
            }
            lplast = p1;
        } else {
            p0 = p1 = lplast;
        }
        lr += 2;
    };
    unsigned s1off = (unsigned)wrap1(2 * j0 - C, Nr2) * (unsigned)Nc2 * 4u;
    const unsigned s1end = (unsigned)Nr2 * (unsigned)Nc2 * 4u;
    unsigned s2off = (unsigned)j0 * (unsigned)Nc4 * 4u;
    (void)trash;
    const int hand_sb = __builtin_amdgcn_readfirstlane((W > 1 && kw > 0) ? 0 : -1);
    CASC_TRACE(1);
    static_for<NV>([&](auto K) { asm_drain1(v[decltype(K)::value]); });
    CASC_TRACE(2);
    auto a1_row = [&](auto A, int sb) {
            constexpr int a = decltype(A)::value;
            constexpr int u = a % (HLEN / 2);
            constexpr int s0 = (2 * u + HLEN - 2) % HLEN, s1 = (2 * u + HLEN - 1) % HLEN;
            const int n = sb * HLEN + a;
            constexpr int r0 = (2 * a) % NV, r1 = r0 + 1;
            int nq1 = n, nq2 = n;
            asm("" : "+s"(nq1));
            asm("" : "+s"(nq2));
            if (nq2 < lim2) {
                if (nq1 < lim1) {
                    asm_wait2<casc_fwd_after<DIST>((a + HLEN - DIST) % HLEN)>(v[r0], v[r1]);
                    row_pass1(v[r0], ring[s0]);
                    row_pass1(v[r1], ring[s1]);
                } else {
                    if constexpr (W > 1) {
                        const int i0 = 2 * (n - NL1);
                        const v4f q0 = *lds_ring(lds_rd, i0), q1 = *lds_ring(lds_rd, i0 + 1);
                        ring[s0][0] = v2f{q0.x, q0.y};
                        ring[s0][1] = v2f{q0.z, q0.w};
                        ring[s1][0] = v2f{q1.x, q1.y};
                        ring[s1][1] = v2f{q1.z, q1.w};
                    }
                }
                {
                    const char *p0, *p1;
                    next_rows(p0, p1);
                    asm_load_s(v[r0], reinterpret_cast<const float*>(p0), xoff);
                    asm_load_s(v[r1], reinterpret_cast<const float*>(p1), xoff);
                }
                v2f ah[2], vd[2];
#pragma unroll
                for (int p = 0; p < 2; p++) ah[p] = vd[p] = v2f{0.f, 0.f};
                static_for<HLEN>([&](auto J) {
                    constexpr int j = decltype(J)::value;
                    constexpr int s = (2 * u + j) % HLEN;
                    const v2f t = f.t[HLEN - 1 - j];
#pragma unroll
                    for (int p = 0; p < 2; p++) {
                        ah[p] = pk_fma(splat(ring[s][p].x), t, ah[p]);
                        vd[p] = pk_fma(splat(ring[s][p].y), t, vd[p]);
                    }
                });
                {
                    asm_store3_sm(b.H1, b.V1, b.D1, off1 + s1off, v2f{ah[0].y, ah[1].y}, v2f{vd[0].x, vd[1].x}, v2f{vd[0].y, vd[1].y},
                                  n < NA ? vmask : 0ull);
                    s1off += (unsigned)Nc2 * 4u;
                    if (s1off == s1end) s1off = 0;
                }
                row_pass2(ah[0].x, ah[1].x, ring2[a]);
                if constexpr (W > 1 && a < HLEN - 2) {
                    if (sb == hand_sb) *lds_ring2(lds_wr, a) = ring2[a];
                }
            } else {
                if constexpr (W > 1) ring2[a] = *lds_ring2(lds_rd, min(n - NA, HLEN - 3));
            }
            if constexpr (a & 1) {
                v2f ah2 = {0.f, 0.f}, vd2 = {0.f, 0.f};
                static_for<HLEN>([&](auto J) {
                    constexpr int j = decltype(J)::value;
                    constexpr int s = (a + 1 + j) % HLEN;
                    const v2f t = f.t[HLEN - 1 - j];
                    ah2 = pk_fma(splat(ring2[s].x), t, ah2);
                    vd2 = pk_fma(splat(ring2[s].y), t, vd2);
                });
                const bool own = (unsigned)(n - (HLEN - 1)) < (unsigned)(2 * rows2);
                asm_store4_sm(b.A2, b.H2, b.V2, b.D2, off2 + s2off, ah2.x, ah2.y, vd2.x, vd2.y, own ? vmask : 0ull);
                s2off += own ? (unsigned)Nc4 * 4u : 0u;
            }
    };
    auto epilogue = [&]() __attribute__((always_inline)) {
        CASC_TRACE(5);
#ifdef PDWT_CASC_TRACE
        asm volatile("s_waitcnt vmcnt(0)" ::: "memory");
#endif
        CASC_TRACE(6);
        CASC_TRACE_STORE(trash, blockIdx.x * W + kw, ((unsigned long long)NA1 << 32) | (unsigned)rows2);
    };
    if constexpr (SPEC) {
        static_assert(W == 16 && (NV == 2 || NV == 4), "wave programs exist for the 16-wave workgroups");
        const unsigned xoff_odd = xoff + (unsigned)strideB;
        auto spec = [&](auto R2c, auto LASTc) __attribute__((always_inline)) {
            constexpr int R2 = decltype(R2c)::value;
            constexpr bool LV = decltype(LASTc)::value;
            using S = CascSpec<HLEN, R2, LV, DIST>;
            constexpr int sNA = S::NA, sNA1 = S::NA1, sNL1 = S::NL1;
            constexpr int WR = LV ? 4 * R2 + 3 * C : 3 * C;
            const bool wraps = LV ? (j0 + R2 == Nr4) : (j0 == 0);
            const size_t wrapB = wraps ? (size_t)Nr * strideB : (size_t)0;
            const unsigned s1wrap = (!LV && j0 == 0) ? s1end : 0u;
            const char* sp = lp;
            static_for<sNA1>([&](auto Nn) {
                constexpr int n = decltype(Nn)::value;
                constexpr int a = n % HLEN;
                constexpr bool from_mem = LV ? true : (n < sNL1);
                constexpr bool computed = LV ? true : (n < sNA);
                constexpr bool store1 = n < sNA;
                constexpr int s0 = (2 * n + HLEN - 2) % HLEN, s1 = (2 * n + HLEN - 1) % HLEN;
                if constexpr (computed) {
                    if constexpr (from_mem) {
                        constexpr int q0 = (2 * n) % NV, q1 = q0 + 1;
                        if constexpr (n >= DIST) asm_wait2<S::wait_cnt(n)>(v[q0], v[q1]);
                        row_pass1(v[q0], ring[s0]);
                        row_pass1(v[q1], ring[s1]);
                        if constexpr (n + DIST < S::LIM) {
                            constexpr int r0 = 2 * (n + DIST) + HLEN - 2;
                            asm volatile("" : "=v"(v[q0]));
                            asm volatile("" : "=v"(v[q1]));
                            asm_load_s(v[q0], reinterpret_cast<const float*>(sp), xoff);
                            if constexpr (r0 + 1 == WR) {
                                asm_load_s(v[q1], reinterpret_cast<const float*>(sp + strideB - wrapB), xoff);
                            } else {
                                asm_load_s(v[q1], reinterpret_cast<const float*>(sp), xoff_odd);
                            }
                            sp += 2 * strideB;
                            if constexpr (r0 + 1 == WR || r0 + 2 == WR) sp -= wrapB;
                        }
                    } else {
                        constexpr int i0 = 2 * (n - sNL1);
                        const v4f q0 = *lds_ring(lds_rd, i0), q1 = *lds_ring(lds_rd, i0 + 1);
                        ring[s0][0] = v2f{q0.x, q0.y};
                        ring[s0][1] = v2f{q0.z, q0.w};
                        ring[s1][0] = v2f{q1.x, q1.y};
                        ring[s1][1] = v2f{q1.z, q1.w};
                    }
                    v2f ah[2], vd[2];
#pragma unroll
                    for (int p = 0; p < 2; p++) ah[p] = vd[p] = v2f{0.f, 0.f};
                    if constexpr (HLEN == 8) {
                        constexpr int q = (2 * n) % 8;
#define PDWT_R(j, p) ring[(q + (j)) % 8][p]
                        col_pass8x2<store1>(ah[0], ah[1], vd[0], vd[1], PDWT_R(0, 0), PDWT_R(1, 0), PDWT_R(2, 0), PDWT_R(3, 0), PDWT_R(4, 0), PDWT_R(5, 0), PDWT_R(6, 0),
                                            PDWT_R(7, 0), PDWT_R(0, 1), PDWT_R(1, 1), PDWT_R(2, 1), PDWT_R(3, 1), PDWT_R(4, 1), PDWT_R(5, 1), PDWT_R(6, 1), PDWT_R(7, 1),
                                            f.t[7], f.t[6], f.t[5], f.t[4], f.t[3], f.t[2], f.t[1], f.t[0]);
#undef PDWT_R
                    } else {
                        static_for<HLEN>([&](auto J) {
                            constexpr int j = decltype(J)::value;
                            constexpr int s = (2 * n + j) % HLEN;
                            const v2f t = f.t[HLEN - 1 - j];
#pragma unroll
                            for (int p = 0; p < 2; p++) {
                                ah[p] = pk_fma_vbcast<0, j == 0>(ring[s][p], t, ah[p]);
                                if constexpr (store1) vd[p] = pk_fma_vbcast<1, j == 0>(ring[s][p], t, vd[p]);
                            }
                        });
                    }
                    if constexpr (store1) {
                        asm_store3_sm(b.H1, b.V1, b.D1, off1 + s1off, v2f{ah[0].y, ah[1].y}, v2f{vd[0].x, vd[1].x}, v2f{vd[0].y, vd[1].y}, vmask);
                        s1off += (unsigned)Nc2 * 4u;
                        if constexpr (n == C - 1) s1off -= s1wrap;
                    }
                    row_pass2(ah[0].x, ah[1].x, ring2[a]);
                    if constexpr (n < HLEN - 2) {
                        if (kw > 0) *lds_ring2(lds_wr, n) = ring2[a];
                    }
                } else {
                    ring2[a] = *lds_ring2(lds_rd, n - sNA);
                }
                if constexpr ((n & 1) && n >= HLEN - 1) {
                    v2f ah2 = {0.f, 0.f}, vd2 = {0.f, 0.f};
                    if constexpr (HLEN == 8) {
                        constexpr int q = (a + 1) % 8;
                        col_pass8x1(ah2, vd2, ring2[q], ring2[(q + 1) % 8], ring2[(q + 2) % 8], ring2[(q + 3) % 8], ring2[(q + 4) % 8], ring2[(q + 5) % 8],
                                    ring2[(q + 6) % 8], ring2[(q + 7) % 8], f.t[7], f.t[6], f.t[5], f.t[4], f.t[3], f.t[2], f.t[1], f.t[0]);
                    } else {
                        static_for<HLEN>([&](auto J) {
                            constexpr int j = decltype(J)::value;
                            constexpr int s = (a + 1 + j) % HLEN;
                            const v2f t = f.t[HLEN - 1 - j];
                            ah2 = pk_fma_vbcast<0, j == 0>(ring2[s], t, ah2);
                            vd2 = pk_fma_vbcast<1, j == 0>(ring2[s], t, vd2);
                        });
                    }
                    asm_store4_sm(b.A2, b.H2, b.V2, b.D2, off2 + s2off, ah2.x, ah2.y, vd2.x, vd2.y, vmask);
                    s2off += (unsigned)Nc4 * 4u;
                }
                if constexpr (n == HLEN / 2 - 1 || n == HLEN - 1) asm volatile("s_waitcnt lgkmcnt(0)\n\ts_barrier" ::: "memory");

#ifdef PDWT_CASC_TRACE
                if constexpr (n == HLEN / 2 - 1) CASC_TRACE(3);
                if constexpr (n == HLEN - 1) CASC_TRACE(4);
#endif
            });
        };
        const int variant = __builtin_amdgcn_readfirstlane(last ? 3 : (rows2 == 5 ? 2 : 1));
        if (variant == 1) {
            spec(std::integral_constant<int, 4>{}, std::false_type{});
            epilogue();
            __builtin_amdgcn_endpgm();
        }
        if (variant == 2) {
            spec(std::integral_constant<int, 5>{}, std::false_type{});
            epilogue();
            __builtin_amdgcn_endpgm();
        }
        spec(std::integral_constant<int, 1>{}, std::true_type{});
        epilogue();
    } else {
    for (int sb = 0;; sb++) {
        static_for<HLEN / 2>([&](auto U) { a1_row(std::integral_constant<int, decltype(U)::value>{}, sb); });
        if constexpr (W > 1) {
            if (sb == 0) asm volatile("s_waitcnt lgkmcnt(0)\n\ts_barrier" ::: "memory");
        }
#ifdef PDWT_CASC_TRACE
        if (sb == 0) CASC_TRACE(3);
#endif
        if (sb * HLEN + HLEN / 2 >= NA1) break;
        static_for<HLEN / 2>([&](auto U) { a1_row(std::integral_constant<int, decltype(U)::value + HLEN / 2>{}, sb); });
        if constexpr (W > 1) {
            if (sb == 0) asm volatile("s_waitcnt lgkmcnt(0)\n\ts_barrier" ::: "memory");
        }
#ifdef PDWT_CASC_TRACE
        if (sb == 0) CASC_TRACE(4);
#endif
        if (sb * HLEN + HLEN >= NA1) break;
    }
    static_for<NV>([&](auto K) { asm_drain1(v[decltype(K)::value]); });
    epilogue();
    }
}

template <int HLEN, int PFD>
__global__ __launch_bounds__(256) void k_inv2d_casc(CascInvBands b, float* __restrict__ out, int Nr, int Nc, int VL,
                                                     float* __restrict__ trash, CascMap cm, Taps2<float> f)
{
    using G = CascInvGeom<HLEN>;
    constexpr int H2 = G::H2, C = G::C, SHIFT = G::SHIFT, NB1 = G::NB1, NB2 = G::NB2, NBT = G::NBT, WIN1 = G::WIN1, WIN2 = G::WIN2;
    constexpr int VM_PF = PFD * (4 + 2 * (3 + 2));
    static_assert(VM_PF - 3 <= 63, "vmcnt is a 6-bit counter");
    static_assert(H2 % PFD == 0 || PFD % H2 == 0, "register slots must be compile-time constants");
    const int lane = threadIdx.x & 63;
    const int xcd = blockIdx.x & 7;
    const int wi = (blockIdx.x >> 3) * 4 + __builtin_amdgcn_readfirstlane(threadIdx.x >> 6);
    if (wi >= cm.cpx * cm.strips) return;
    const int cy = xcd * cm.cpx + wi / cm.strips;
    const int strip = wi % cm.strips;
    const int Nr1 = Nr >> 1, Nc1 = Nc >> 1, Nr2 = Nr >> 2, Nc2 = Nc >> 2;
    const int nchunks = 8 * cm.cpx;
    const int ya = G::BASE + 2 * (int)(((long long)cy * (Nr1 >> 1)) / nchunks);
    const int ye = G::BASE + 2 * (int)(((long long)(cy + 1) * (Nr1 >> 1)) / nchunks);
    const int rows1 = ye - ya;
    if (rows1 <= 0) return;
    const int cx1 = strip * VL * 2 + 2 * (lane - NBT);
    const bool valid = (lane >= NBT) && (lane < NBT + VL) && (cx1 < Nc1);
    const int cx1w = wrapi(cx1, Nc1);
    const int cx2w = cx1w >> 1;
    const int gA = ya - C;
    const int P0 = (gA + SHIFT) >> 1;
    const int r2base = P0 - C;
    const int nrows1 = rows1 + H2 - 1 + SHIFT;
    const int nsteps = (nrows1 + 1) >> 1;

    const float* const pA2 = b.A2 + cx2w;
    const float* const pH2 = b.H2 + cx2w;
    const float* const pV2 = b.V2 + cx2w;
    const float* const pD2 = b.D2 + cx2w;
    const float* const pH1 = b.H1 + cx1w;
    const float* const pV1 = b.V1 + cx1w;
    const float* const pD1 = b.D1 + cx1w;
    auto off2 = [&](int r2) { return (size_t)wrap1(r2base + r2, Nr2) * Nc2; };
    auto off1 = [&](int r1) { return (size_t)wrap1(gA + r1, Nr1) * Nc1; };
    const unsigned voff2 = (unsigned)cx2w * 4u, voff1 = (unsigned)cx1w * 4u, voffo = (unsigned)(valid ? cx1 : 0) * 8u;
    const lanemask_t vmask = __ballot(valid);

    v2f r2av[H2], r2hd[H2];
    v2f ra[H2], rh[H2], rv[H2], rd[H2];
#pragma unroll
    for (int k = 0; k < H2; k++) ra[k] = rh[k] = rv[k] = rd[k] = v2f{0.f, 0.f};
    float q2[PFD][4];
    v2f q1[2 * PFD][3];
    {
#pragma unroll
        for (int r = 0; r < H2 - 1; r++) {
            const size_t o = off2(r);
            r2av[r] = v2f{pA2[o], pV2[o]};
            r2hd[r] = v2f{pH2[o], pD2[o]};
        }
        r2av[H2 - 1] = r2hd[H2 - 1] = v2f{0.f, 0.f};
#pragma unroll
        for (int p = 0; p < PFD; p++) {
            const size_t o = off2(H2 - 1 + p);
            q2[p][0] = pA2[o];
            q2[p][1] = pH2[o];
            q2[p][2] = pV2[o];
            q2[p][3] = pD2[o];
        }
#pragma unroll
        for (int q = 0; q < 2 * PFD; q++) {
            const size_t o = off1(q);
            q1[q][0] = *reinterpret_cast<const v2f*>(pH1 + o);
            q1[q][1] = *reinterpret_cast<const v2f*>(pV1 + o);
            q1[q][2] = *reinterpret_cast<const v2f*>(pD1 + o);
        }
    }

    float* const tr = trash + (size_t)(blockIdx.x & 7) * Nc;

    auto emit = [&](auto S0, auto OFF, int g) {
        constexpr int s0 = decltype(S0)::value, off = decltype(OFF)::value;
        const bool own = (g >= 0) && (g < 2 * rows1);
        float o4[4] = {0.f, 0.f, 0.f, 0.f};
        if (own) {
            v2f sa = {0.f, 0.f}, sh = {0.f, 0.f}, sv = {0.f, 0.f}, sd = {0.f, 0.f};
            static_for<H2>([&](auto J) {
                constexpr int j = decltype(J)::value;
                constexpr int s = (s0 + j) % H2;
                constexpr int k = HLEN - 1 - (2 * j + off);
                constexpr int kp = k & ~1;
                const v2f pl2 = v2f{f.a[kp], f.a[kp + 1]}, ph2 = v2f{f.b[kp], f.b[kp + 1]};
                sa = pk_fma_sbcast<k & 1, false>(ra[s], pl2, sa);
                sh = pk_fma_sbcast<k & 1, false>(rh[s], ph2, sh);
                sv = pk_fma_sbcast<k & 1, false>(rv[s], pl2, sv);
                sd = pk_fma_sbcast<k & 1, false>(rd[s], ph2, sd);
            });
            const v2f t1o = sa + sh, t2o = sv + sd;
            float t1[WIN1], t2[WIN1];
            t1[NB1 * 2] = t1o.x;
            t1[NB1 * 2 + 1] = t1o.y;
            t2[NB1 * 2] = t2o.x;
            t2[NB1 * 2 + 1] = t2o.y;
    #pragma unroll
            for (int k = 0; k < NB1; k++) {
                const int dl = (NB1 - 1 - k) * 2, sl = (NB1 - k) * 2, dr = (NB1 + 1 + k) * 2, sr = (NB1 + k) * 2;
    #pragma unroll
                for (int cc = 0; cc < 2; cc++) {
                    t1[dl + cc] = dpp_shr1(t1[sl + cc]);
                    t2[dl + cc] = dpp_shr1(t2[sl + cc]);
                    t1[dr + cc] = dpp_shl1(t1[sr + cc]);
                    t2[dr + cc] = dpp_shl1(t2[sr + cc]);
                }
            }
            auto pair_out = [&](auto E0) {
                constexpr int e0 = decltype(E0)::value;
                constexpr int pl = (e0 + SHIFT) >> 1;
                v2f s1 = {0.f, 0.f}, s2 = {0.f, 0.f};
    #pragma unroll
                for (int j = 0; j < H2; j++) {
                    const int m = HLEN - 1 - 2 * j;
                    s1 = pk_fma(splat(t1[NB1 * 2 + pl - C + j]), v2f{f.a[m - 1], f.a[m]}, s1);
                    s2 = pk_fma(splat(t2[NB1 * 2 + pl - C + j]), v2f{f.b[m - 1], f.b[m]}, s2);
                }
                const v2f o = s1 + s2;
                o4[e0] = o.x;
                o4[e0 + 1] = o.y;
            };
            auto single_out = [&](auto E) {
                constexpr int eo = decltype(E)::value;
                constexpr int gp = eo + SHIFT;
                constexpr int pl = gp >> 1, offx = 1 - (gp & 1);
                float s1 = 0.f, s2 = 0.f;
    #pragma unroll
                for (int j = 0; j < H2; j++) {
                    const int k = HLEN - 1 - (2 * j + offx);
                    s1 = __builtin_fmaf(t1[NB1 * 2 + pl - C + j], f.a[k], s1);
                    s2 = __builtin_fmaf(t2[NB1 * 2 + pl - C + j], f.b[k], s2);
                }
                o4[eo] = s1 + s2;
            };
            if constexpr (SHIFT == 0) {
                pair_out(std::integral_constant<int, 0>{});
                pair_out(std::integral_constant<int, 2>{});
            } else {
                single_out(std::integral_constant<int, 0>{});
                pair_out(std::integral_constant<int, 1>{});
                single_out(std::integral_constant<int, 3>{});
            }
        }
        asm_store_sm(own ? out + (size_t)wrap1(2 * ya + g, Nr) * Nc : tr, voffo, v4f{o4[0], o4[1], o4[2], o4[3]}, vmask);
    };

    auto synth2 = [&](auto S0, auto OFF, float& a0, float& a1) {
        constexpr int s0 = decltype(S0)::value, off = decltype(OFF)::value;
        v2f sav = {0.f, 0.f}, shd = {0.f, 0.f};
        static_for<H2>([&](auto J) {
            constexpr int j = decltype(J)::value;
            constexpr int s = (s0 + j) % H2;
            constexpr int k = HLEN - 1 - (2 * j + off);
            constexpr int kp = k & ~1;
            sav = pk_fma_sbcast<k & 1, false>(r2av[s], v2f{f.a[kp], f.a[kp + 1]}, sav);
            shd = pk_fma_sbcast<k & 1, false>(r2hd[s], v2f{f.b[kp], f.b[kp + 1]}, shd);
        });
        const v2f t = sav + shd;
        float t1[WIN2], t2[WIN2];
        t1[NB2] = t.x;
        t2[NB2] = t.y;
#pragma unroll
        for (int k = 0; k < NB2; k++) {
            t1[NB2 - 1 - k] = dpp_shr1(t1[NB2 - k]);
            t2[NB2 - 1 - k] = dpp_shr1(t2[NB2 - k]);
            t1[NB2 + 1 + k] = dpp_shl1(t1[NB2 + k]);
            t2[NB2 + 1 + k] = dpp_shl1(t2[NB2 + k]);
        }
        float o2[2];
#pragma unroll
        for (int e = 0; e < 2; e++) {
            const int gp = e + SHIFT;
            const int pl = gp >> 1, offx = 1 - (gp & 1);
            float s1 = 0.f, s2 = 0.f;
#pragma unroll
            for (int j = 0; j < H2; j++) {
                const int k = HLEN - 1 - (2 * j + offx);
                s1 = __builtin_fmaf(t1[NB2 + pl - C + j], f.a[k], s1);
                s2 = __builtin_fmaf(t2[NB2 + pl - C + j], f.b[k], s2);
            }
            o2[e] = s1 + s2;
        }
        a0 = o2[0];
        a1 = o2[1];
    };

    constexpr int kWait2 = VM_PF - 4, kWait1 = VM_PF - 3;
    auto step = [&](auto Pp, int sb) {
        constexpr int p = decltype(Pp)::value;
        const int s = sb * H2 + p;
        constexpr int pr = p % PFD;
        asm_wait4<kWait2>(q2[pr][0], q2[pr][1], q2[pr][2], q2[pr][3]);
        r2av[(H2 - 1 + p) % H2] = v2f{asm_copy(q2[pr][0]), asm_copy(q2[pr][2])};
        r2hd[(H2 - 1 + p) % H2] = v2f{asm_copy(q2[pr][1]), asm_copy(q2[pr][3])};
        {
            const size_t o = off2(min(H2 - 1 + s + PFD, H2 - 2 + nsteps));
            asm_load_s(q2[pr][0], b.A2 + o, voff2);
            asm_load_s(q2[pr][1], b.H2 + o, voff2);
            asm_load_s(q2[pr][2], b.V2 + o, voff2);
            asm_load_s(q2[pr][3], b.D2 + o, voff2);
        }
        static_for<2>([&](auto I) {
            constexpr int idx = decltype(I)::value;
            constexpr int q = 2 * p + idx;
            float a0, a1;
            synth2(std::integral_constant<int, p % H2>{}, std::integral_constant<int, 1 - idx>{}, a0, a1);
            const int r1 = 2 * s + idx;
            constexpr int qr = q % (2 * PFD);
            asm_wait3<kWait1>(q1[qr][0], q1[qr][1], q1[qr][2]);
            ra[q % H2] = v2f{a0, a1};
            rh[q % H2] = asm_copy(q1[qr][0]);
            rv[q % H2] = asm_copy(q1[qr][1]);
            rd[q % H2] = asm_copy(q1[qr][2]);
            {
                const size_t o = off1(min(r1 + 2 * PFD, 2 * nsteps - 1));
                asm_load_s(q1[qr][0], b.H1 + o, voff1);
                asm_load_s(q1[qr][1], b.V1 + o, voff1);
                asm_load_s(q1[qr][2], b.D1 + o, voff1);
            }
            const int g1 = 2 * (r1 - (H2 - 1)) - SHIFT;
            emit(std::integral_constant<int, (q + 1) % H2>{}, std::integral_constant<int, 1>{}, g1);
            emit(std::integral_constant<int, (q + 1) % H2>{}, std::integral_constant<int, 0>{}, g1 + 1);
        });
    };

    static_for<PFD>([&](auto K) {
        constexpr int k = decltype(K)::value;
        asm_drain1(q2[k][0]);
        asm_drain1(q2[k][1]);
        asm_drain1(q2[k][2]);
        asm_drain1(q2[k][3]);
    });
    static_for<2 * PFD>([&](auto K) {
        constexpr int k = decltype(K)::value;
        asm_drain1(q1[k][0]);
        asm_drain1(q1[k][1]);
        asm_drain1(q1[k][2]);
    });
    for (int sb = 0;; sb++) {
        bool fin = false;
        static_for<H2>([&](auto Pp) {
            if (!fin) {
                step(Pp, sb);
                fin = (sb * H2 + decltype(Pp)::value + 1 >= nsteps);
            }
        });
        if (fin) break;
    }
    static_for<PFD>([&](auto K) {
        constexpr int k = decltype(K)::value;
        asm_drain1(q2[k][0]);
        asm_drain1(q2[k][1]);
        asm_drain1(q2[k][2]);
        asm_drain1(q2[k][3]);
    });
    static_for<2 * PFD>([&](auto K) {
        constexpr int k = decltype(K)::value;
        asm_drain1(q1[k][0]);
        asm_drain1(q1[k][1]);
        asm_drain1(q1[k][2]);
    });
}

#define PDWT_CHECK_LAUNCH() PDWT_HIP_TRY(hipGetLastError())

static bool casc_enabled() { return knob(KN_CASC) == 1; }

template <int HLEN>
static int launch_fwd_casc(const float* in, const CascBands& b, float* trash, int nr, int nc, const Taps2<float>& f2, const CascBatchF* d_tbl, int nimg)
{
    TapsLH f;
    for (int k = 0; k < PDWT_MAX_FILTER_WIDTH; k++) f.t[k] = v2f{f2.a[k], f2.b[k]};
    constexpr int MAXVL = CascGeom<HLEN>::MAXVL;
    const int strips = idiv_up(nc, MAXVL * 4);
    const int VL = idiv_up(nc / 4, strips);
    constexpr int NVD = HLEN > 16 ? 4 : (HLEN % 4 == 0 ? HLEN / 2 : HLEN);
    KTimer kt(K_FWD2D_CASC, true);
    int W = knob(KN_CASC_WG);
    if (W == 0) W = 16;
    if (W != 1 && W != 4 && W != 8 && W != 16) W = 16;
    constexpr size_t REG = casc_fwd_region_bytes<HLEN>();
    while (W > 1 && (size_t)(W - 1) * REG > 150 * 1024) W /= 2;
    if (W == 2) W = 1;
    if (W > 1) {
        const int nr4 = nr / 4;
        const int wgs = knob(KN_CASC_WAVES) > 0 ? idiv_up(knob(KN_CASC_WAVES), W) : 256;
        int gy = std::max(1, wgs / strips);
        while (W > 4 && (nr4 / gy) / W < HLEN / 2) W /= 2;
        while (gy > 1 && (nr4 / gy) / W < HLEN / 2) gy--;
        if (gy >= 1 && (nr4 / gy) / W >= HLEN / 2) {
            int nwg = gy * strips;
            const size_t lds = (size_t)(W - 1) * REG;
            void (*k)(const float*, CascBands, int, int, int, float*, CascMap, TapsLH);
            k = (W == 4) ? k_fwd2d_casc<HLEN, NVD, 4> : (W == 8) ? k_fwd2d_casc<HLEN, NVD, 8> : k_fwd2d_casc<HLEN, NVD, 16>;
            const bool nv2 = W == 16 && (knob(KN_CASC_NV) == 0 || knob(KN_CASC_NV) == 2);
            if (nv2) k = k_fwd2d_casc<HLEN, 2, 16>;
            bool spec = nv2 && (knob(KN_CASC_SPEC) & 1) && 2 * 4 >= HLEN;
            auto spec_ok = [&](int gyq, int xwq) {
                const int cpxq = idiv_up(gyq * strips, 8);
                for (int g = 0; g < gyq; g++)
                    for (int st = 0; st < strips; st++) {
                        const int R = casc_chunk_start(g + 1, st, nr4, gyq, strips, cpxq, xwq) - casc_chunk_start(g, st, nr4, gyq, strips, cpxq, xwq);
                        if (R < 16) return false;
                        const int E = std::min((3 * (HLEN - 2) + 3) / 4, R / 16 - 1);
                        const int base = (R + E) / 16, rem = (R + E) % 16;
                        if (base != 4 || R - (15 * base + std::min(15, rem)) != 1) return false;
                    }
                return true;
            };
            if (spec && (knob(KN_CASC_SPEC) & 4) && knob(KN_CASC_WAVES) <= 0 && !d_tbl && (nr4 / gy) / 16 >= 8) {
                const int gy2 = (nr4 + 36) / 73;
                if (gy2 >= 3 * gy && spec_ok(gy2, 0)) {
                    gy = gy2;
                    nwg = gy * strips;
                }
            }
            int xw = spec ? knob(KN_CASC_XCDW) : 0;
            if (spec && xw != 0 && !spec_ok(gy, xw)) xw = 0;
            spec = spec && spec_ok(gy, xw);
            if (!spec) xw = 0;
            if (spec) {
                k = k_fwd2d_casc<HLEN, 2, 16, true>;
                stat_casc_spec(0);
            }
            const CascMap cm = {idiv_up(nwg, 8), strips, gy, xw, d_tbl};
            const dim3 grid((unsigned)(8 * cm.cpx), (unsigned)(d_tbl ? nimg : 1));
            if (lds > 64 * 1024) {
                int rc = (W == 4) ? lds_opt_in<k_fwd2d_casc<HLEN, NVD, 4>>()
                         : (W == 8) ? lds_opt_in<k_fwd2d_casc<HLEN, NVD, 8>>() : lds_opt_in<k_fwd2d_casc<HLEN, NVD, 16>>();
                if (rc == PDWT_OK && nv2) rc = lds_opt_in<k_fwd2d_casc<HLEN, 2, 16>>();
                if (rc == PDWT_OK && spec) rc = lds_opt_in<k_fwd2d_casc<HLEN, 2, 16, true>>();
                if (rc != PDWT_OK) return rc;
            }
            PDWT_LAUNCH_KT(kt, k, grid, dim3(64 * W), lds, in, b, nr, nc, VL, trash, cm, f);
            PDWT_CHECK_LAUNCH();
            return PDWT_OK;
        }
    }
    if (d_tbl) return 1;
    int cpx = (knob(KN_CASC_WAVES) > 0 ? knob(KN_CASC_WAVES) : 1024) / (8 * strips);
    if (cpx > nr / 4 / 4 / 8) cpx = nr / 4 / 4 / 8;
    if (cpx < 1) cpx = 1;
    const CascMap cm = {cpx, strips, 0};
    const dim3 grid((unsigned)(8 * idiv_up(cpx * strips, 4)));
    const int nv = knob(KN_CASC_NV) > 0 ? knob(KN_CASC_NV) : NVD;
    if (nv == 2)
        PDWT_LAUNCH_KT(kt, (k_fwd2d_casc<HLEN, 2, 1>), grid, dim3(256), 0, in, b, nr, nc, VL, trash, cm, f);
    else if (nv < HLEN && HLEN % 4 == 0)
        PDWT_LAUNCH_KT(kt, (k_fwd2d_casc<HLEN, NVD, 1>), grid, dim3(256), 0, in, b, nr, nc, VL, trash, cm, f);
    else
        PDWT_LAUNCH_KT(kt, (k_fwd2d_casc<HLEN, (HLEN > 16 ? NVD : HLEN), 1>), grid, dim3(256), 0, in, b, nr, nc, VL, trash, cm, f);
    PDWT_CHECK_LAUNCH();
    return PDWT_OK;
}

#ifdef PDWT_CASC_ONLY8
#define PDWT_CASC_FWD_HLENS(X) X(8)
#else
#define PDWT_CASC_FWD_HLENS(X) X(4) X(6) X(8) X(10) X(12) X(14) X(16) X(18) X(20)
#endif

int fwd2d_casc_f32(const float* in, float* H1, float* V1, float* D1, float* A2, float* H2, float* V2, float* D2, float* trash, int nr,
                   int nc, int hlen, const Taps2<float>& f, const CascBatchF* d_tbl, int nimg)
{
    if (!casc_enabled() || !stream_enabled() || !trash) return 1;
    if ((nr & 3) || (nc & 3) || nc < 256 || nr < 16 * hlen) return 1;
    if ((long long)nr * nc < (long long)knob(KN_CASC_MIN)) return 1;
    if ((long long)nr * nc >= (1LL << 32)) return 1;
    if (!al16(in) || !al16(H1) || !al16(V1) || !al16(D1) || !al16(A2) || !al16(H2) || !al16(V2) || !al16(D2)) return 1;
    const CascBands b = {H1, V1, D1, A2, H2, V2, D2};
    switch (hlen) {
#define X(H) \
    case H: return launch_fwd_casc<H>(in, b, trash, nr, nc, f, d_tbl, nimg);
        PDWT_CASC_FWD_HLENS(X)
#undef X
        default: return 1;
    }
}

template <int HLEN>
static int launch_inv_casc(const CascInvBands& b, float* out, float* trash, int nr, int nc, const Taps2<float>& f)
{
    constexpr int MAXVL = CascInvGeom<HLEN>::MAXVL;
    const int nc1 = nc / 2;
    const int strips = idiv_up(nc1, MAXVL * 2);
    const int VL = idiv_up(nc1 / 2, strips);
    int cpx = (knob(KN_CASC_IWAVES) > 0 ? knob(KN_CASC_IWAVES) : 2048) / (8 * strips);
    if (cpx > nr / 2 / 8 / 8) cpx = nr / 2 / 8 / 8;
    if (cpx < 1) cpx = 1;
    const CascMap cm = {cpx, strips, 0};
    const dim3 grid((unsigned)(8 * idiv_up(cpx * strips, 4)));
    KTimer kt(K_INV2D_CASC, true);
    constexpr int H2 = HLEN / 2;
    const int pfd = knob(KN_CASC_IPFD);
    bool launched = false;
    if constexpr (H2 % 2 == 0) {
        if (pfd == 2) {
            PDWT_LAUNCH_KT(kt, (k_inv2d_casc<HLEN, 2>), grid, dim3(256), 0, b, out, nr, nc, VL, trash, cm, f);
            launched = true;
        }
    }
    if constexpr (H2 * 14 - 3 <= 63 && H2 > 2) {
        if (pfd >= H2 && !launched) {
            PDWT_LAUNCH_KT(kt, (k_inv2d_casc<HLEN, H2>), grid, dim3(256), 0, b, out, nr, nc, VL, trash, cm, f);
            launched = true;
        }
    }
    if (!launched) PDWT_LAUNCH_KT(kt, (k_inv2d_casc<HLEN, 1>), grid, dim3(256), 0, b, out, nr, nc, VL, trash, cm, f);
    PDWT_CHECK_LAUNCH();
    return PDWT_OK;
}

#ifdef PDWT_CASC_ONLY8
#define PDWT_CASC_INV_HLENS(X) X(8)
#else
#define PDWT_CASC_INV_HLENS(X) X(4) X(6) X(8) X(10)
#endif

int inv2d_casc_f32(const float* A2, const float* H2, const float* V2, const float* D2, const float* H1, const float* V1, const float* D1,
                   float* out, float* trash, int nr, int nc, int hlen, const Taps2<float>& f)
{
    if (!casc_enabled() || !stream_enabled() || !trash) return 1;
    if ((nr & 3) || (nc & 3) || nc < 256 || nr < 32 * hlen) return 1;
    if ((long long)nr * nc < (long long)knob(KN_CASC_MIN)) return 1;
    if (!al16(out) || !al16(H1) || !al16(V1) || !al16(D1) || !al16(A2) || !al16(H2) || !al16(V2) || !al16(D2) || !al16(trash)) return 1;
    const CascInvBands b = {A2, H2, V2, D2, H1, V1, D1};
    switch (hlen) {
#define X(H) \
    case H: return launch_inv_casc<H>(b, out, trash, nr, nc, f);
        PDWT_CASC_INV_HLENS(X)
#undef X
        default: return 1;
    }
}

}
```

### pdwt_amd/csrc/dwt_casc.hpp

```cpp
#pragma once
#include "common.hpp"
#include "casc_dev.hpp"

namespace pdwt {
int fwd2d_casc_f32(const float* in, float* H1, float* V1, float* D1, float* A2, float* H2, float* V2, float* D2, float* trash, int nr,
                   int nc, int hlen, const Taps2<float>& f, const CascBatchF* d_tbl = nullptr, int nimg = 1);
int inv2d_casc_f32(const float* A2, const float* H2, const float* V2, const float* D2, const float* H1, const float* V1, const float* D1,
                   float* out, float* trash, int nr, int nc, int hlen, const Taps2<float>& f);
}
```

### pdwt_amd/csrc/runtime.hip

```cpp
#include <set>
#include <utility>
#include <stdio.h>
#include <stdlib.h>
#include <string.h>

#include <mutex>
#include <vector>

#include "common.hpp"

namespace pdwt {

static thread_local char g_err[512] = "";

void set_last_error(hipError_t e, const char* what, const char* file, int line)
{
    snprintf(g_err, sizeof(g_err), "%s: %s (%s:%d)", hipGetErrorString(e), what, file, line);
    (void)hipGetLastError();
}

static std::mutex g_mu;
static hipStream_t g_streams[64] = {};
static hipStream_t g_user_streams[64] = {};
static bool g_user_set[64] = {};

hipStream_t stream()
{
    int dev = 0;
    if (hipGetDevice(&dev) != hipSuccess || dev < 0 || dev >= 64) return nullptr;
    std::lock_guard<std::mutex> lk(g_mu);
    if (g_user_set[dev]) return g_user_streams[dev];
    if (!g_streams[dev]) {
        static const bool nonblocking = getenv("PDWT_STREAM_NONBLOCKING") && atoi(getenv("PDWT_STREAM_NONBLOCKING")) == 1;
        if (hipStreamCreateWithFlags(&g_streams[dev], nonblocking ? hipStreamNonBlocking : hipStreamDefault) != hipSuccess) {
            g_streams[dev] = nullptr;
        }
    }
    return g_streams[dev];
}

int lds_opt_in_ptr(const void* kernel)
{
    static std::mutex mu;
    static std::set<std::pair<const void*, int>> done;
    int dev = 0;
    PDWT_HIP_TRY(hipGetDevice(&dev));
    std::lock_guard<std::mutex> lk(mu);
    if (done.count({kernel, dev})) return PDWT_OK;
    PDWT_HIP_TRY(hipFuncSetAttribute(kernel, hipFuncAttributeMaxDynamicSharedMemorySize, 160 * 1024));
    done.insert({kernel, dev});
    return PDWT_OK;
}

struct KnobDef { const char* name; const char* env; int dflt; };
static const KnobDef g_knob_defs[KN_COUNT] = {
    {"force_twopass", "PDWT_FORCE_TWOPASS", 0}, {"tiled_cols", "PDWT_TILED_COLS", 0},
    {"casc", "PDWT_CASC", 1}, {"casc_waves", "PDWT_CASC_WAVES", 0}, {"casc_nv", "PDWT_CASC_NV", 0},
    {"casc_min", "PDWT_CASC_MIN", 2048 * 2048}, {"casc_iwaves", "PDWT_CASC_IWAVES", 0}, {"casc_ipfd", "PDWT_CASC_IPFD", 1},
    {"casc_wg", "PDWT_CASC_WG", 0}, {"casc_iwg", "PDWT_CASC_IWG", 0}, {"casc_l3", "PDWT_CASC_L3", 1}, {"casc_spec", "PDWT_CASC_SPEC", 7}, {"casc_xcdw", "PDWT_CASC_XCDW", 0}, {"dwt1d_lds_kb", "PDWT_DWT1D_LDS_KB", 80},
    {"stream", "PDWT_STREAM", 1}, {"stream_r", "PDWT_STREAM_R", 0}, {"stream_waves", "PDWT_STREAM_WAVES", 8192},
    {"stream_narrow", "PDWT_STREAM_NARROW", 2048 * 2048}, {"small", "PDWT_SMALL", 1},
    {"rows_tr", "PDWT_ROWS_TR", 1}, {"ring_r", "PDWT_RING_R", 0}, {"ring_waves", "PDWT_RING_WAVES", 4096},
    {"swtf", "PDWT_SWTF", 1}, {"swtf_m", "PDWT_SWTF_M", 0}, {"swtf_mi", "PDWT_SWTF_MI", 0},
    {"swtf_xcd", "PDWT_SWTF_XCD", 1}, {"swtf_alt", "PDWT_SWTF_ALT", 1}, {"swtf_perm", "PDWT_SWTF_PERM", 1}, {"swtf_f64", "PDWT_SWTF_F64", 1},
    {"f64_lds", "PDWT_F64_LDS", 1}, {"f64_lds_min", "PDWT_F64_LDS_MIN", 256}, {"f64_lds_wgs", "PDWT_F64_LDS_WGS", 512}, {"f64_lds_mingroups", "PDWT_F64_LDS_MINGROUPS", 1}, {"f64_lds_skew", "PDWT_F64_LDS_SKEW", 64}, {"norm2sq_ref1d", "PDWT_NORM2SQ_REF1D", 0},
    {"norm_in_threshold", "PDWT_NORM_IN_THRESHOLD", -1},
    {"selfcheck", "PDWT_SELFCHECK", 1}, {"dwt1d_f64", "PDWT_DWT1D_F64", 1}, {"swtf_long", "PDWT_SWTF_LONG", 1}, {"f64_tail", "PDWT_F64_TAIL", 0},
    {"exp0", "PDWT_EXP0", 0}, {"exp1", "PDWT_EXP1", 0}, {"exp2", "PDWT_EXP2", 0}, {"exp3", "PDWT_EXP3", 0}, {"nonsep_tiled", "PDWT_NONSEP_TILED", 1},
    {"f64_lat", "PDWT_F64_LAT", 1}, {"f64_lat_min", "PDWT_F64_LAT_MIN", 4096}, {"dwt1d_nt_mb", "PDWT_DWT1D_NT_MB", 192},
};
static int g_knob_vals[KN_COUNT];
static std::once_flag g_knob_once;
static void knob_init()
{
    for (int i = 0; i < KN_COUNT; i++) {
        const char* e = getenv(g_knob_defs[i].env);
        g_knob_vals[i] = (e && *e) ? atoi(e) : g_knob_defs[i].dflt;
    }
}
int knob(KnobId id)
{
    std::call_once(g_knob_once, knob_init);
    return g_knob_vals[id];
}
int knob_set(const char* name, int value)
{
    std::call_once(g_knob_once, knob_init);
    if (!name) return PDWT_EINVAL;
    for (int i = 0; i < KN_COUNT; i++) {
        if (!strcmp(name, g_knob_defs[i].name)) {
            g_knob_vals[i] = value;
            return PDWT_OK;
        }
    }
    return PDWT_EINVAL;
}

std::atomic<int> g_stat_spec_fwd{0}, g_stat_spec_inv{0};
void stat_casc_spec(int inverse) { (inverse ? g_stat_spec_inv : g_stat_spec_fwd).fetch_add(1, std::memory_order_relaxed); }
std::atomic<int> g_stat_lat_fwd{0}, g_stat_lat_inv{0};
void stat_lat(int inverse) { (inverse ? g_stat_lat_inv : g_stat_lat_fwd).fetch_add(1, std::memory_order_relaxed); }

int knob_get(const char* name, int* value)
{
    std::call_once(g_knob_once, knob_init);
    if (!name || !value) return PDWT_EINVAL;
    if (!strcmp(name, "stat_casc_spec_fwd") || !strcmp(name, "stat_casc_spec_inv")) {
        *value = (name[15] == 'f' ? g_stat_spec_fwd : g_stat_spec_inv).load(std::memory_order_relaxed);
        return PDWT_OK;
    }
    if (!strcmp(name, "stat_lat_fwd") || !strcmp(name, "stat_lat_inv")) {
        *value = (name[9] == 'f' ? g_stat_lat_fwd : g_stat_lat_inv).load(std::memory_order_relaxed);
        return PDWT_OK;
    }
    for (int i = 0; i < KN_COUNT; i++) {
        if (!strcmp(name, g_knob_defs[i].name)) {
            *value = g_knob_vals[i];
            return PDWT_OK;
        }
    }
    return PDWT_EINVAL;
}

static unsigned long long* g_probe[64] = {};
static unsigned long long* g_probe_allbuf[64] = {};
static bool g_probe_on = false;
static int g_probe_all = 0;
unsigned long long* clock_probe_all(int* all)
{
    *all = 0;
    if (!g_probe_all) return nullptr;
    int dev = 0;
    if (hipGetDevice(&dev) != hipSuccess || dev < 0 || dev >= 64) return nullptr;
    if (!g_probe_allbuf[dev] && hipMalloc(&g_probe_allbuf[dev], (size_t)kClockProbeAllBlocks * 4 * sizeof(unsigned long long)) != hipSuccess) return nullptr;
    *all = g_probe_all;
    return g_probe_allbuf[dev];
}
unsigned long long* clock_probe_slot(int slot)
{
    if (!g_probe_on || slot < 0 || slot >= 16) return nullptr;
    int dev = 0;
    if (hipGetDevice(&dev) != hipSuccess || dev < 0 || dev >= 64) return nullptr;
    if (!g_probe[dev]) {
        if (hipMalloc(&g_probe[dev], 16 * 4 * sizeof(unsigned long long)) != hipSuccess) return nullptr;
        (void)hipMemsetAsync(g_probe[dev], 0, 16 * 4 * sizeof(unsigned long long), stream());
    }
    return g_probe[dev] + 4 * slot;
}

static const char* const g_knames[K_COUNT] = {
    "fwd2d_fused", "inv2d_fused", "ana_rows", "ana_cols", "syn_cols", "syn_rows",
    "swt_ana_rows", "swt_ana_cols", "swt_syn_cols", "swt_syn_rows",
    "haar2d_fwd", "haar2d_inv", "haar1d_fwd", "haar1d_inv", "soft_thresh", "abs_sum", "abs_sum_final",
    "fwd2d_casc", "inv2d_casc", "fwd2d_stream", "inv2d_stream", "fwd2d_small", "inv2d_small", "fwd2d_f64", "inv2d_f64", "thresh_sum",
};
struct KRec { int id; hipEvent_t e0, e1; };
static thread_local bool g_kt_on = false;
static thread_local std::vector<KRec>* g_kt = nullptr;
static thread_local std::vector<hipEvent_t>* g_evpool = nullptr;

static hipEvent_t ev_get()
{
    if (g_evpool && !g_evpool->empty()) {
        hipEvent_t e = g_evpool->back();
        g_evpool->pop_back();
        return e;
    }
    hipEvent_t e = nullptr;
    if (hipEventCreate(&e) != hipSuccess) return nullptr;
    return e;
}

KTimer::KTimer(int kernel_id, bool attach_to_launch) : id(kernel_id), ext(attach_to_launch)
{
    if (!g_kt_on) return;
    e0 = ev_get();
    e1 = ev_get();
    if (e0 && !ext) (void)hipEventRecord(e0, stream());
}
KTimer::~KTimer()
{
    if (!e0 || !e1) return;
    if (!ext) (void)hipEventRecord(e1, stream());
    if (!g_kt) g_kt = new std::vector<KRec>();
    g_kt->push_back(KRec{id, e0, e1});
}

}

using namespace pdwt;

extern "C" {

int pdwt_device_count(void)
{
    int n = 0;
    if (hipGetDeviceCount(&n) != hipSuccess) {
        (void)hipGetLastError();
        return 0;
    }
    return n;
}
int pdwt_set_device(int dev)
{
    PDWT_HIP_TRY(hipSetDevice(dev));
    return PDWT_OK;
}
int pdwt_get_device(void)
{
    int dev = -1;
    if (hipGetDevice(&dev) != hipSuccess) return PDWT_EHIP;
    return dev;
}
int pdwt_device_name(char* buf, int buflen)
{
    if (!buf || buflen <= 0) return PDWT_EINVAL;
    int dev = 0;
    PDWT_HIP_TRY(hipGetDevice(&dev));
    hipDeviceProp_t p;
    PDWT_HIP_TRY(hipGetDeviceProperties(&p, dev));
    snprintf(buf, (size_t)buflen, "%s (%s, %d CUs)", p.name, p.gcnArchName, p.multiProcessorCount);
    return PDWT_OK;
}
void* pdwt_malloc(size_t nbytes)
{
    void* p = nullptr;
    hipError_t e = hipMalloc(&p, nbytes ? nbytes : 1);
    if (e != hipSuccess) {
        set_last_error(e, "hipMalloc", __FILE__, __LINE__);
        return nullptr;
    }
    return p;
}
int pdwt_free(void* dptr)
{
    if (!dptr) return PDWT_OK;
    PDWT_HIP_TRY(hipStreamSynchronize(stream()));
    PDWT_HIP_TRY(hipFree(dptr));
    return PDWT_OK;
}
int pdwt_memset(void* dptr, int byte, size_t nbytes)
{
    if (!nbytes) return PDWT_OK;
    PDWT_HIP_TRY(hipMemsetAsync(dptr, byte, nbytes, stream()));
    return PDWT_OK;
}
int pdwt_memcpy_h2d(void* dst, const void* src, size_t nbytes)
{
    if (!nbytes) return PDWT_OK;
    PDWT_HIP_TRY(hipMemcpyAsync(dst, src, nbytes, hipMemcpyHostToDevice, stream()));
    PDWT_HIP_TRY(hipStreamSynchronize(stream()));
    return PDWT_OK;
}
int pdwt_memcpy_d2h(void* dst, const void* src, size_t nbytes)
{
    if (!nbytes) return PDWT_OK;
    PDWT_HIP_TRY(hipMemcpyAsync(dst, src, nbytes, hipMemcpyDeviceToHost, stream()));
    PDWT_HIP_TRY(hipStreamSynchronize(stream()));
    return PDWT_OK;
}
int pdwt_memcpy_d2d(void* dst, const void* src, size_t nbytes)
{
    if (!nbytes) return PDWT_OK;
    PDWT_HIP_TRY(hipMemcpyAsync(dst, src, nbytes, hipMemcpyDeviceToDevice, stream()));
    return PDWT_OK;
}
int pdwt_memcpy_d2d_foreign(void* dst, const void* src, size_t nbytes)
{
    if (!nbytes) return PDWT_OK;
    PDWT_HIP_TRY(hipStreamSynchronize(nullptr));
    PDWT_HIP_TRY(hipMemcpyAsync(dst, src, nbytes, hipMemcpyDeviceToDevice, stream()));
    PDWT_HIP_TRY(hipStreamSynchronize(stream()));
    return PDWT_OK;
}
int pdwt_sync(void)
{
    PDWT_HIP_TRY(hipStreamSynchronize(stream()));
    return PDWT_OK;
}
void* pdwt_get_stream(void) { return (void*)stream(); }
int pdwt_set_stream(void* user_stream, int use_it)
{
    int dev = 0;
    PDWT_HIP_TRY(hipGetDevice(&dev));
    if (dev < 0 || dev >= 64) return PDWT_EINVAL;
    PDWT_HIP_TRY(hipStreamSynchronize(stream()));
    std::lock_guard<std::mutex> lk(g_mu);
    g_user_set[dev] = use_it != 0;
    g_user_streams[dev] = use_it ? (hipStream_t)user_stream : nullptr;
    return PDWT_OK;
}
const char* pdwt_last_error_string(void) { return g_err; }

void* pdwt_event_create(void)
{
    hipEvent_t e = nullptr;
    if (hipEventCreate(&e) != hipSuccess) return nullptr;
    return (void*)e;
}
int pdwt_event_record(void* ev)
{
    PDWT_HIP_TRY(hipEventRecord((hipEvent_t)ev, stream()));
    return PDWT_OK;
}
int pdwt_event_sync(void* ev)
{
    PDWT_HIP_TRY(hipEventSynchronize((hipEvent_t)ev));
    return PDWT_OK;
}
float pdwt_event_elapsed_ms(void* a, void* b)
{
    float ms = -1.f;
    if (hipEventElapsedTime(&ms, (hipEvent_t)a, (hipEvent_t)b) != hipSuccess) return -1.f;
    return ms;
}
int pdwt_event_destroy(void* ev)
{
    PDWT_HIP_TRY(hipEventDestroy((hipEvent_t)ev));
    return PDWT_OK;
}

int pdwt_graph_allowed(void) { return (g_kt_on || g_probe_on) ? 0 : 1; }
int pdwt_graph_capture_begin(void)
{
    (void)pdwt::counted_waits_ok();
    PDWT_HIP_TRY(hipStreamBeginCapture(pdwt::stream(), hipStreamCaptureModeThreadLocal));
    return PDWT_OK;
}
int pdwt_graph_capture_end(void** exec_out)
{
    if (!exec_out) return PDWT_EINVAL;
    *exec_out = nullptr;
    hipGraph_t g = nullptr;
    hipError_t e = hipStreamEndCapture(pdwt::stream(), &g);
    if (e != hipSuccess || !g) {
        (void)hipGetLastError();
        return PDWT_EHIP;
    }
    hipGraphExec_t x = nullptr;
    e = hipGraphInstantiate(&x, g, nullptr, nullptr, 0);
    (void)hipGraphDestroy(g);
    if (e != hipSuccess || !x) {
        (void)hipGetLastError();
        return PDWT_EHIP;
    }
    *exec_out = (void*)x;
    return PDWT_OK;
}
int pdwt_graph_launch(void* exec)
{
    if (!exec) return PDWT_EINVAL;
    PDWT_HIP_TRY(hipGraphLaunch((hipGraphExec_t)exec, pdwt::stream()));
    return PDWT_OK;
}
int pdwt_graph_destroy(void* exec)
{
    if (exec) PDWT_HIP_TRY(hipGraphExecDestroy((hipGraphExec_t)exec));
    return PDWT_OK;
}

namespace {
typedef float probe_v4f __attribute__((ext_vector_type(4)));
__global__ __launch_bounds__(256) void k_bw_probe(const probe_v4f* __restrict__ in, probe_v4f* __restrict__ out, size_t n4, int mode)
{
    const size_t G = gridDim.x, nblk = (n4 + 255) / 256, per = (nblk + G - 1) / G;
    probe_v4f acc = {0.f, 0.f, 0.f, 0.f};
    for (size_t k = 0; k < per; k += 8) {
        probe_v4f r[8];
        size_t idx[8];
        bool on[8];
#pragma unroll
        for (int u = 0; u < 8; u++) {
            idx[u] = (blockIdx.x * per + k + u) * 256 + threadIdx.x;
            on[u] = (k + u < per) && idx[u] < n4;
            if (mode != 2) r[u] = in[on[u] ? idx[u] : threadIdx.x];
            else r[u] = probe_v4f{1.f, 2.f, 3.f, (float)u};
        }
#pragma unroll
        for (int u = 0; u < 8; u++) {
            if (mode == 1) acc += r[u];
            else if (on[u]) out[idx[u]] = r[u];
        }
    }
    if (mode == 1 && acc.x + acc.y + acc.z + acc.w == 12345.678f) out[0] = acc;
}
}
int pdwt_probe_bandwidth(const void* src, void* dst, size_t bytes, int mode)
{
    if (mode < 0 || mode > 2 || bytes < 4096 || (mode != 2 && !src) || !dst) return PDWT_EINVAL;
    int dev = 0, ncu = 256;
    PDWT_HIP_TRY(hipGetDevice(&dev));
    PDWT_HIP_TRY(hipDeviceGetAttribute(&ncu, hipDeviceAttributeMultiprocessorCount, dev));
    hipLaunchKernelGGL(k_bw_probe, dim3((unsigned)(8 * ncu)), dim3(256), 0, pdwt::stream(), (const probe_v4f*)src, (probe_v4f*)dst, bytes / 16, mode);
    PDWT_HIP_TRY(hipGetLastError());
    return PDWT_OK;
}

int pdwt_clock_probe_enable(int on)
{
    g_probe_on = on == 1;
    g_probe_all = on >= 2 ? on - 1 : 0;
    return PDWT_OK;
}
int pdwt_clock_probe_dump(unsigned long long* out, int nblocks)
{
    int dev = 0;
    PDWT_HIP_TRY(hipGetDevice(&dev));
    if (!out || nblocks < 1 || nblocks > kClockProbeAllBlocks || dev < 0 || dev >= 64 || !g_probe_allbuf[dev]) return PDWT_EINVAL;
    return pdwt_memcpy_d2h(out, g_probe_allbuf[dev], (size_t)nblocks * 4 * sizeof(unsigned long long));
}
int pdwt_clock_probe_read(int slot, double* shader_mhz, double* span_us)
{
    if (slot < 0 || slot >= 16 || !shader_mhz || !span_us) return PDWT_EINVAL;
    int dev = 0;
    PDWT_HIP_TRY(hipGetDevice(&dev));
    *shader_mhz = *span_us = 0.0;
    if (dev < 0 || dev >= 64 || !g_probe[dev]) return PDWT_OK;
    unsigned long long h[4];
    const int rc = pdwt_memcpy_d2h(h, g_probe[dev] + 4 * slot, sizeof(h));
    if (rc != PDWT_OK) return rc;
    if (h[3] > h[1] && h[2] > h[0]) {
        const double ticks = (double)(h[3] - h[1]);
        *span_us = ticks / 100.0;
        *shader_mhz = (double)(h[2] - h[0]) / ticks * 100.0;
    }
    return PDWT_OK;
}
int pdwt_ktime_enable(int on)
{
    g_kt_on = on != 0;
    return PDWT_OK;
}
int pdwt_ktime_reset(void)
{
    if (g_kt) {
        if (!g_evpool) g_evpool = new std::vector<hipEvent_t>();
        (void)hipStreamSynchronize(stream());
        for (auto& r : *g_kt) {
            g_evpool->push_back(r.e0);
            g_evpool->push_back(r.e1);
        }
        g_kt->clear();
    }
    return PDWT_OK;
}
int pdwt_ktime_read(int kernel_id, int* n_launches, double* total_ms)
{
    if (kernel_id < 0 || kernel_id >= K_COUNT) return PDWT_EINVAL;
    PDWT_HIP_TRY(hipStreamSynchronize(stream()));
    int n = 0;
    double tot = 0;
    if (g_kt) {
        for (auto& r : *g_kt) {
            if (r.id != kernel_id) continue;
            float ms = 0;
            if (hipEventElapsedTime(&ms, r.e0, r.e1) == hipSuccess) {
                tot += ms;
                n++;
            }
        }
    }
    if (n_launches) *n_launches = n;
    if (total_ms) *total_ms = tot;
    return PDWT_OK;
}
const char* pdwt_kernel_name(int kernel_id) { return (kernel_id >= 0 && kernel_id < K_COUNT) ? g_knames[kernel_id] : nullptr; }
int pdwt_kernel_count(void) { return K_COUNT; }

}
```

Before: 343,000 Mpixels/s.

## Fuse level-3 forward DWT into cascaded two-level kernel with ticketed halo completion

```diff
diff --git a/pdwt_amd/csrc/casc_dev.hpp b/pdwt_amd/csrc/casc_dev.hpp
--- a/pdwt_amd/csrc/casc_dev.hpp
+++ b/pdwt_amd/csrc/casc_dev.hpp
@@ -45,6 +45,19 @@
 struct CascBatchF {
     const float* in;
     CascBands b;
+};
+
+struct CascL3 {
+    float *A3, *H3, *V3, *D3;
+    unsigned* tickets;
+    const void* tbl;
+};
+void casc_l3_prepare();
+bool user_stream_set();
+struct CascL3Req {
+    float *A3, *H3, *V3, *D3;
+    const void* tbl;
+    bool done;
 };
 
 template <int HLEN>
diff --git a/pdwt_amd/csrc/common.hpp b/pdwt_amd/csrc/common.hpp
--- a/pdwt_amd/csrc/common.hpp
+++ b/pdwt_amd/csrc/common.hpp
@@ -146,6 +146,7 @@
     KN_F64_LAT,
     KN_F64_LAT_MIN,
     KN_DWT1D_NT_MB,
+    KN_CASC_L3F,
     KN_COUNT
 };
 int knob(KnobId id);
diff --git a/pdwt_amd/csrc/dwt.hip b/pdwt_amd/csrc/dwt.hip
--- a/pdwt_amd/csrc/dwt.hip
+++ b/pdwt_amd/csrc/dwt.hip
@@ -627,8 +627,16 @@
             if (lev + 1 < w.nlevels && !force_twopass()) {
                 T* a2 = (lev + 2 == w.nlevels) ? c[0] : s.ping[pp];
                 float* trash = s.t1_is_trash ? (float*)s.t1 : nullptr;
+                CascL3Req l3 = {nullptr, nullptr, nullptr, nullptr, nullptr, false};
+                const bool offer3 = lev == 0 && lev + 2 < w.nlevels;
+                if (offer3) {
+                    l3.A3 = (lev + 3 == w.nlevels) ? c[0] : s.ping[pp ^ 1];
+                    l3.H3 = c[3 * lev + 7];
+                    l3.V3 = c[3 * lev + 8];
+                    l3.D3 = c[3 * lev + 9];
+                }
                 rc = fwd2d_casc_f32(in, c[3 * lev + 1], c[3 * lev + 2], c[3 * lev + 3], a2, c[3 * lev + 4], c[3 * lev + 5], c[3 * lev + 6],
-                                    trash, nr, nc, w.hlen, f);
+                                    trash, nr, nc, w.hlen, f, nullptr, 1, offer3 ? &l3 : nullptr);
                 if (rc < 0) return rc;
                 if (rc == PDWT_OK) {
                     in = a2;
@@ -636,6 +644,13 @@
                     nr = div2(div2(nr));
                     nc = div2(div2(nc));
                     lev++;
+                    if (l3.done) {
+                        in = l3.A3;
+                        pp ^= 1;
+                        nr = div2(nr);
+                        nc = div2(nc);
+                        lev++;
+                    }
                     continue;
                 }
             }
@@ -940,10 +955,11 @@
     int lev0 = 0;
     if (B->d_cf && B->trash0) {
         const CascBands& b = B->cf0.b;
+        CascL3Req l3 = {nullptr, nullptr, nullptr, nullptr, B->w.nlevels >= 3 ? (const void*)(B->d_fwd + (size_t)2 * B->nimg) : nullptr, false};
         const int rc = fwd2d_casc_f32(B->cf0.in, b.H1, b.V1, b.D1, b.A2, b.H2, b.V2, b.D2, B->trash0, B->lev_nr[0], B->lev_nc[0], B->w.hlen, f,
-                                      B->d_cf, B->nimg);
+                                      B->d_cf, B->nimg, B->w.nlevels >= 3 ? &l3 : nullptr);
         if (rc < 0) return rc;
-        if (rc == PDWT_OK) lev0 = 2;
+        if (rc == PDWT_OK) lev0 = l3.done ? 3 : 2;
     }
     for (int lev = lev0; lev < B->w.nlevels; lev++) {
         const int rc = fwd2d_stream_batch_f32(B->d_fwd + (size_t)lev * B->nimg, B->nimg, B->trash_floats, B->lev_nr[lev], B->lev_nc[lev], B->w.hlen, f);
diff --git a/pdwt_amd/csrc/dwt_casc.hip b/pdwt_amd/csrc/dwt_casc.hip
--- a/pdwt_amd/csrc/dwt_casc.hip
+++ b/pdwt_amd/csrc/dwt_casc.hip
@@ -1,6 +1,8 @@
 #include "dwt_casc.hpp"
 
 #include <algorithm>
+#include <cstddef>
+#include <mutex>
 
 #include "dwt_stream.hpp"
 #include "stream_dev.hpp"
@@ -72,11 +74,11 @@
         : "v"(a0), "v"(a1), "v"(a2), "v"(a3), "v"(a4), "v"(a5), "v"(a6), "v"(a7), "s"(t0), "s"(t1), "s"(t2), "s"(t3), "s"(t4), "s"(t5), "s"(t6), "s"(t7));
 }
 
-template <int HLEN, int R2, bool LV, int DIST>
+template <int HLEN, int R2, bool LV, int DIST, int S2 = 4>
 struct CascSpec {
     static constexpr int NA = 2 * R2, NA1 = NA + HLEN - 2, NL1 = NA - HLEN / 2 + 1;
     static constexpr int LIM = LV ? NA1 : NL1;
-    static constexpr int stores_at(int q) { return ((q < NA) ? 3 : 0) + (((q & 1) && q >= HLEN - 1) ? 4 : 0); }
+    static constexpr int stores_at(int q) { return ((q < NA) ? 3 : 0) + (((q & 1) && q >= HLEN - 1) ? S2 : 0); }
     static constexpr int loads_at(int q) { return (q < LIM && q + DIST < LIM) ? 2 : 0; }
     static constexpr int wait_cnt(int n)
     {
@@ -87,10 +89,254 @@
     }
 };
 
-template <int HLEN, int NV, int W, bool SPEC = false>
-__global__ __launch_bounds__(W == 1 ? 256 : 64 * W) void k_fwd2d_casc(const float* in, CascBands b, int Nr, int Nc, int VL,
-                                                                       float* __restrict__ trash, CascMap cm, TapsLH f)
-{
+__device__ __forceinline__ void asm_store3f_sm(float* b0, float* b1, float* b2, unsigned voff, float d0, float d1, float d2, lanemask_t mask)
+{
+    lanemask_t saved;
+    asm volatile("s_and_saveexec_b64 %0, %8\n\tglobal_store_dword %1, %2, %5\n\tglobal_store_dword %1, %3, %6\n\tglobal_store_dword %1, %4, %7\n\ts_mov_b64 exec, %0"
+                 : "=&s"(saved) : "v"(voff), "v"(d0), "v"(d1), "v"(d2), "s"(b0), "s"(b1), "s"(b2), "s"(mask) : "memory", "scc");
+}
+
+struct Casc3fArgs {
+    const float* in;
+    CascBands b;
+    int Nr, Nc, VL;
+    float* trash;
+    CascMap cm;
+    TapsLH f;
+    CascL3 l3;
+};
+static_assert(sizeof(CascL3) == 6 * sizeof(void*), "six 8-byte words");
+typedef v2f __attribute__((aligned(4))) v2f_a4;
+typedef float __attribute__((address_space(1))) casc_gf32;
+typedef unsigned __attribute__((address_space(1))) casc_gu32;
+constexpr size_t kL3BandBytes = 1024 * 2 * sizeof(v2f);
+struct CascL3Starts {
+    int lr0, lc0;
+    int nOr, nOc;
+    int nIr, nIc;
+};
+template <int HLEN>
+__host__ __device__ inline CascL3Starts casc_l3_starts(int J0, int R, int c0, int VLt)
+{
+    constexpr int C = HLEN / 2 - 1;
+    CascL3Starts s;
+    s.lr0 = (J0 + C) & 1;
+    s.lc0 = (c0 + C) & 1;
+    s.nOr = (R - s.lr0 + 1) >> 1;
+    s.nOc = (VLt - s.lc0 + 1) >> 1;
+    s.nIr = (R - HLEN - s.lr0 + 2) >> 1;
+    s.nIc = (VLt - HLEN - s.lc0 + 2) >> 1;
+    if (s.nIr < 0) s.nIr = 0;
+    if (s.nIc < 0) s.nIc = 0;
+    return s;
+}
+__device__ __forceinline__ void asm_store_sm_sc1(const void* sbase, unsigned voff, float d, lanemask_t mask)
+{
+    lanemask_t saved;
+    asm volatile("s_and_saveexec_b64 %0, %4\n\tglobal_store_dword %1, %2, %3 sc1\n\ts_mov_b64 exec, %0"
+                 : "=&s"(saved) : "v"(voff), "v"(d), "s"(sbase), "s"(mask) : "memory", "scc");
+}
+__device__ __forceinline__ unsigned asm_ticket_add(const void* sbase, unsigned voff, lanemask_t mask)
+{
+    lanemask_t saved;
+    unsigned old;
+    const unsigned one = 1u;
+    asm volatile("s_and_saveexec_b64 %0, %5\n\tglobal_atomic_add %1, %2, %3, %4 sc0\n\ts_waitcnt vmcnt(0)\n\ts_mov_b64 exec, %0"
+                 : "=&s"(saved), "=&v"(old) : "v"(voff), "v"(one), "s"(sbase), "s"(mask) : "memory", "scc");
+    return old;
+}
+template <int HLEN>
+__device__ __forceinline__ void casc_l3_store(const CascL3& l3, int r0, int cc0, int Nr8, int Nc8, v2f ah, v2f vd)
+{
+    constexpr int C = HLEN / 2 - 1;
+    int i3 = (r0 + C) >> 1, j3 = (cc0 + C) >> 1;
+    i3 = i3 >= Nr8 ? i3 - Nr8 : i3;
+    j3 = j3 >= Nc8 ? j3 - Nc8 : j3;
+    const size_t oo = (size_t)i3 * Nc8 + j3;
+    l3.A3[oo] = ah.x;
+    l3.H3[oo] = ah.y;
+    l3.V3[oo] = vd.x;
+    l3.D3[oo] = vd.y;
+}
+#ifdef PDWT_CASC_TRACE
+#define CASC_L3_TRACE_PARAM , unsigned long long* tr_
+#define CASC_L3_TRACE_ARG , casc_tr_
+#define CASC_L3_MARK(i) tr_[i] = wall_clock64()
+#else
+#define CASC_L3_TRACE_PARAM
+#define CASC_L3_TRACE_ARG
+#define CASC_L3_MARK(i)
+#endif
+template <int HLEN>
+__device__ __forceinline__ void casc_fwd_l3_tail(const float* tile, unsigned* flag, const TapsLH& f, int kw, int lane CASC_L3_TRACE_PARAM)
+{
+    typedef const unsigned long long __attribute__((address_space(4))) * ka_t;
+    typedef const int __attribute__((address_space(4))) * kai_t;
+    const char __attribute__((address_space(4))) * ka = (const char __attribute__((address_space(4)))*)__builtin_amdgcn_kernarg_segment_ptr();
+    asm volatile("" : "+s"(ka));
+    const int Nr4 = ((kai_t)(ka + offsetof(Casc3fArgs, Nr)))[0] >> 2, Nc4 = ((kai_t)(ka + offsetof(Casc3fArgs, Nc)))[0] >> 2;
+    const int VL = ((kai_t)(ka + offsetof(Casc3fArgs, VL)))[0];
+    CascMap cm;
+    {
+        const kai_t q = (kai_t)(ka + offsetof(Casc3fArgs, cm));
+        cm = CascMap{q[0], q[1], q[2], q[3], (const void*)((ka_t)(ka + offsetof(Casc3fArgs, cm) + offsetof(CascMap, tbl)))[0]};
+    }
+    const int wg = ((int)blockIdx.x & 7) * cm.cpx + ((int)blockIdx.x >> 3);
+    const int g = wg / cm.strips, strip = wg - g * cm.strips;
+    const int J0 = casc_chunk_start(g, strip, Nr4, cm.gy, cm.strips, cm.cpx, 0);
+    const int R = casc_chunk_start(g + 1, strip, Nr4, cm.gy, cm.strips, cm.cpx, 0) - J0;
+    float* A2 = (float*)((ka_t)(ka + offsetof(Casc3fArgs, b.A2)))[0];
+    CascL3 l3;
+    {
+        const ka_t q = (ka_t)(ka + offsetof(Casc3fArgs, l3));
+        l3 = CascL3{(float*)q[0], (float*)q[1], (float*)q[2], (float*)q[3], (unsigned*)q[4], (const void*)q[5]};
+    }
+    if (cm.tbl) {
+        static_assert(sizeof(StreamBatchF) == 6 * sizeof(void*) && sizeof(CascBatchF) == 8 * sizeof(void*), "pointer tables");
+        A2 = (float*)((ka_t)(const unsigned long long*)cm.tbl + 8 * (size_t)blockIdx.y)[4];
+        const ka_t q3 = (ka_t)(const unsigned long long*)l3.tbl + 6 * (size_t)blockIdx.y;
+        l3.A3 = (float*)q3[1];
+        l3.H3 = (float*)q3[2];
+        l3.V3 = (float*)q3[3];
+        l3.D3 = (float*)q3[4];
+    }
+    using G = CascGeom<HLEN>;
+    constexpr int NBT = G::NBT, E = HLEN - 1;
+    const int Nr8 = Nr4 >> 1, Nc8 = Nc4 >> 1;
+    const int c0 = strip * VL, VLt = min(VL, Nc4 - c0);
+    const int tid = kw * 64 + lane;
+    asm volatile("s_waitcnt lgkmcnt(0)\n\ts_barrier" ::: "memory");
+    CASC_L3_MARK(1);
+    {
+        const int lc = lane - NBT;
+        const bool cval = lc >= 0 && lc < VLt;
+        const lanemask_t m_row = __ballot(cval), m_col = __ballot(cval && (lc < E || lc >= VLt - E));
+        const unsigned voff = (unsigned)(cval ? c0 + lc : 0) * 4u;
+        for (int lr = kw; lr < R; lr += 16) {
+            const bool redge = lr < E || lr >= R - E;
+            asm_store_sm_sc1(A2 + (size_t)(J0 + lr) * Nc4, voff, tile[lr * 64 + lane], redge ? m_row : m_col);
+        }
+    }
+    {
+        const CascL3Starts s = casc_l3_starts<HLEN>(J0, R, c0, VLt);
+        const int nI = s.nIr * s.nIc;
+        for (int ob = 0; ob < nI; ob += 1024) {
+            const int o = min(ob + tid, nI - 1);
+            const int ir = o / s.nIc, ic = o - ir * s.nIc;
+            const int lr = s.lr0 + 2 * ir, lc = s.lc0 + 2 * ic;
+            const float* const p = tile + lr * 64 + NBT + lc;
+            v2f rp[HLEN];
+            static_for<HLEN>([&](auto K) {
+                constexpr int k = decltype(K)::value;
+                v2f acc = {0.f, 0.f};
+                static_for<HLEN / 2>([&](auto J) {
+                    constexpr int j = 2 * decltype(J)::value;
+                    const v2f w = *reinterpret_cast<const v2f_a4*>(p + k * 64 + j);
+                    acc = pk_fma_vbcast<0, j == 0>(w, f.t[HLEN - 1 - j], acc);
+                    acc = pk_fma_vbcast<1, false>(w, f.t[HLEN - 2 - j], acc);
+                });
+                rp[k] = acc;
+            });
+            v2f ah = {0.f, 0.f}, vd = {0.f, 0.f};
+            static_for<HLEN>([&](auto K) {
+                constexpr int k = decltype(K)::value;
+                ah = pk_fma_vbcast<0, k == 0>(rp[k], f.t[HLEN - 1 - k], ah);
+                vd = pk_fma_vbcast<1, k == 0>(rp[k], f.t[HLEN - 1 - k], vd);
+            });
+            casc_l3_store<HLEN>(l3, J0 + lr, c0 + lc, Nr8, Nc8, ah, vd);
+        }
+    }
+    CASC_L3_MARK(2);
+    asm volatile("s_waitcnt vmcnt(0) lgkmcnt(0)\n\ts_barrier" ::: "memory");
+    CASC_L3_MARK(3);
+    if (kw == 0) {
+        int tg = g - (lane & 1), ts = strip - ((lane >> 1) & 1);
+        tg = tg < 0 ? tg + cm.gy : tg;
+        ts = ts < 0 ? ts + cm.strips : ts;
+        const unsigned voff = (unsigned)(((int)blockIdx.y * cm.gy + tg) * cm.strips + ts) * 4u;
+        const unsigned old = asm_ticket_add(l3.tickets, voff, 0xfull);
+        const lanemask_t lastm = __ballot(old == 3u) & 0xfull;
+        asm_store_sm_sc1(l3.tickets, voff, 0.f, lastm);
+        flag[0] = (unsigned)lastm;
+    }
+    asm volatile("s_waitcnt vmcnt(0) lgkmcnt(0)\n\ts_barrier" ::: "memory");
+    const unsigned mine = (unsigned)__builtin_amdgcn_readfirstlane((int)flag[0]);
+    CASC_L3_MARK(4);
+    __builtin_amdgcn_fence(__ATOMIC_ACQUIRE, "wavefront");
+    constexpr int BW = 2 * E;
+    constexpr int BST = 64 + 8, RST = 2 * HLEN;
+    static_assert((BW * BST + 99 * RST) * sizeof(float) <= kL3BandBytes && BW <= 16, "the bands fit the tile's place; one band row per wave");
+    float* const bandB = const_cast<float*>(tile);
+    float* const bandR = bandB + BW * BST;
+    for (int q = 0; q < 4; q++) {
+        if (!((mine >> q) & 1u)) continue;
+        int tg = g - (q & 1), ts = strip - (q >> 1);
+        tg = tg < 0 ? tg + cm.gy : tg;
+        ts = ts < 0 ? ts + cm.strips : ts;
+        const int qJ0 = casc_chunk_start(tg, ts, Nr4, cm.gy, cm.strips, cm.cpx, 0);
+        const int qR = casc_chunk_start(tg + 1, ts, Nr4, cm.gy, cm.strips, cm.cpx, 0) - qJ0;
+        const int qc0 = ts * VL, qVL = min(VL, Nc4 - qc0);
+        const CascL3Starts s = casc_l3_starts<HLEN>(qJ0, qR, qc0, qVL);
+        const int wq = s.nOc - s.nIc;
+        const int nB = (s.nOr - s.nIr) * s.nOc;
+        const int nS = nB + s.nIr * wq;
+        {
+            const int bi = min(kw, BW - 1);
+            const casc_gf32* const brow = (const casc_gf32*)A2 + (size_t)wrap1(qJ0 + qR - E + bi, Nr4) * Nc4;
+            const int bj0 = lane, bj1 = min(64 + lane, qVL + E - 1);
+            const int nR = qR * BW;
+            int ri[2], rj[2];
+            float v[4];
+#pragma unroll
+            for (int u = 0; u < 2; u++) {
+                const int idx = min(tid + 1024 * u, nR - 1);
+                ri[u] = idx / BW;
+                rj[u] = idx - ri[u] * BW;
+            }
+            v[0] = __hip_atomic_load(brow + wrap1(qc0 + bj0, Nc4), __ATOMIC_RELAXED, __HIP_MEMORY_SCOPE_AGENT);
+            v[1] = __hip_atomic_load(brow + wrap1(qc0 + bj1, Nc4), __ATOMIC_RELAXED, __HIP_MEMORY_SCOPE_AGENT);
+#pragma unroll
+            for (int u = 0; u < 2; u++)
+                v[2 + u] = __hip_atomic_load((const casc_gf32*)A2 + ((unsigned)(qJ0 + ri[u]) * (unsigned)Nc4 + (unsigned)wrap1(qc0 + qVL - E + rj[u], Nc4)),
+                                             __ATOMIC_RELAXED, __HIP_MEMORY_SCOPE_AGENT);
+            bandB[bi * BST + bj0] = v[0];
+            bandB[bi * BST + bj1] = v[1];
+#pragma unroll
+            for (int u = 0; u < 2; u++) bandR[ri[u] * RST + rj[u]] = v[2 + u];
+        }
+        asm volatile("s_waitcnt lgkmcnt(0)\n\ts_barrier" ::: "memory");
+        for (int ob = 0; ob < nS; ob += 1024) {
+            const int o = min(ob + tid, nS - 1);
+            const int irB = o / s.nOc, o2 = max(o - nB, 0), irR = o2 / wq;
+            const bool lower = o < nB;
+            const int ir = lower ? irB + s.nIr : irR;
+            const int ic = lower ? o - irB * s.nOc : o2 - irR * wq + s.nIc;
+            const int lr = s.lr0 + 2 * ir, lc = s.lc0 + 2 * ic;
+            const float* const p = lower ? bandB + (lr - (qR - E)) * BST + lc : bandR + lr * RST + (lc - (qVL - E));
+            const int st = lower ? BST : RST;
+            v2f ah = {0.f, 0.f}, vd = {0.f, 0.f};
+            static_for<HLEN>([&](auto K) {
+                constexpr int k = decltype(K)::value;
+                v2f acc = {0.f, 0.f};
+                static_for<HLEN / 2>([&](auto J) {
+                    constexpr int j = 2 * decltype(J)::value;
+                    const v2f w = *reinterpret_cast<const v2f_a4*>(p + k * st + j);
+                    acc = pk_fma_vbcast<0, j == 0>(w, f.t[HLEN - 1 - j], acc);
+                    acc = pk_fma_vbcast<1, false>(w, f.t[HLEN - 2 - j], acc);
+                });
+                ah = pk_fma_vbcast<0, k == 0>(acc, f.t[HLEN - 1 - k], ah);
+                vd = pk_fma_vbcast<1, k == 0>(acc, f.t[HLEN - 1 - k], vd);
+            });
+            casc_l3_store<HLEN>(l3, qJ0 + lr, qc0 + lc, Nr8, Nc8, ah, vd);
+        }
+        asm volatile("s_waitcnt lgkmcnt(0)\n\ts_barrier" ::: "memory");
+    }
+}
+
+template <int HLEN, int NV, int W, bool SPEC, bool L3F>
+__device__ __forceinline__ void casc_fwd_body(const float* in, CascBands b, int Nr, int Nc, int VL, float* __restrict__ trash, CascMap cm, TapsLH f)
+{
+    static_assert(!L3F || (SPEC && W == 16), "the level-3 tail exists for the wave programs");
     using G = CascGeom<HLEN>;
     constexpr int C = G::C, NB1 = G::NB1, NB2 = G::NB2, NBT = G::NBT, WIN1 = G::WIN1, WIN2 = G::WIN2;
     extern __shared__ __attribute__((aligned(16))) unsigned char lds_raw[];
@@ -109,6 +355,7 @@
     const int Nc2 = Nc >> 1, Nr2 = Nr >> 1, Nr4 = Nr >> 2, Nc4 = Nc >> 2;
     const int kw = __builtin_amdgcn_readfirstlane(threadIdx.x >> 6);
     int j0, rows2, strip;
+    int tJ0 = 0;
     bool last;
     if constexpr (W == 1) {
         const int xcd = blockIdx.x & 7;
@@ -135,6 +382,7 @@
         rows2 = (kw < W - 1) ? base + (kw < rem ? 1 : 0) : R - start;
         j0 = J0 + start;
         last = (kw == W - 1);
+        tJ0 = J0;
     }
     const int xs = strip * VL * 4;
     const int x = xs + 4 * (lane - NBT);
@@ -160,6 +408,9 @@
     unsigned char* const lds_wr = lds_raw + (size_t)(W > 1 && kw > 0 ? kw - 1 : 0) * REG;
     auto lds_ring = [&](unsigned char* reg, int r) { return reinterpret_cast<v4f*>(reg + ((size_t)r * 64 + lane) * 16); };
     auto lds_ring2 = [&](unsigned char* reg, int r) { return reinterpret_cast<v2f*>(reg + (size_t)(HLEN - 2) * 64 * 16 + ((size_t)r * 64 + lane) * 8); };
+    unsigned* const l3_flag = reinterpret_cast<unsigned*>(lds_raw + (size_t)(W - 1) * REG);
+    float* const l3_tile = reinterpret_cast<float*>(lds_raw + (size_t)(W - 1) * REG + 16);
+    float* const l3_wr = l3_tile + (size_t)(j0 - tJ0) * 64 + lane;
     auto row_pass1 = [&](const v4f& v, v2f (&lh)[2]) {
         float w[WIN1];
 #pragma unroll
@@ -330,7 +581,7 @@
             }
     };
     auto epilogue = [&]() __attribute__((always_inline)) {
-        CASC_TRACE(5);
+        if constexpr (!L3F) CASC_TRACE(5);
 #ifdef PDWT_CASC_TRACE
         asm volatile("s_waitcnt vmcnt(0)" ::: "memory");
 #endif
@@ -343,7 +594,7 @@
         auto spec = [&](auto R2c, auto LASTc) __attribute__((always_inline)) {
             constexpr int R2 = decltype(R2c)::value;
             constexpr bool LV = decltype(LASTc)::value;
-            using S = CascSpec<HLEN, R2, LV, DIST>;
+            using S = CascSpec<HLEN, R2, LV, DIST, L3F ? 3 : 4>;
             constexpr int sNA = S::NA, sNA1 = S::NA1, sNL1 = S::NL1;
             constexpr int WR = LV ? 4 * R2 + 3 * C : 3 * C;
             const bool wraps = LV ? (j0 + R2 == Nr4) : (j0 == 0);
@@ -433,7 +684,12 @@
                             vd2 = pk_fma_vbcast<1, j == 0>(ring2[s], t, vd2);
                         });
                     }
-                    asm_store4_sm(b.A2, b.H2, b.V2, b.D2, off2 + s2off, ah2.x, ah2.y, vd2.x, vd2.y, vmask);
+                    if constexpr (L3F) {
+                        l3_wr[((n - (HLEN - 1)) / 2) * 64] = ah2.x;
+                        asm_store3f_sm(b.H2, b.V2, b.D2, off2 + s2off, ah2.y, vd2.x, vd2.y, vmask);
+                    } else {
+                        asm_store4_sm(b.A2, b.H2, b.V2, b.D2, off2 + s2off, ah2.x, ah2.y, vd2.x, vd2.y, vmask);
+                    }
                     s2off += (unsigned)Nc4 * 4u;
                 }
                 if constexpr (n == HLEN / 2 - 1 || n == HLEN - 1) asm volatile("s_waitcnt lgkmcnt(0)\n\ts_barrier" ::: "memory");
@@ -445,17 +701,24 @@
             });
         };
         const int variant = __builtin_amdgcn_readfirstlane(last ? 3 : (rows2 == 5 ? 2 : 1));
+        auto l3_tail = [&]() __attribute__((always_inline)) {
+            if constexpr (L3F) CASC_TRACE(5);
+            if constexpr (L3F) casc_fwd_l3_tail<HLEN>(l3_tile, l3_flag, f, kw, lane CASC_L3_TRACE_ARG);
+        };
         if (variant == 1) {
             spec(std::integral_constant<int, 4>{}, std::false_type{});
+            l3_tail();
             epilogue();
             __builtin_amdgcn_endpgm();
         }
         if (variant == 2) {
             spec(std::integral_constant<int, 5>{}, std::false_type{});
+            l3_tail();
             epilogue();
             __builtin_amdgcn_endpgm();
         }
         spec(std::integral_constant<int, 1>{}, std::true_type{});
+        l3_tail();
         epilogue();
     } else {
     for (int sb = 0;; sb++) {
@@ -479,6 +742,20 @@
     static_for<NV>([&](auto K) { asm_drain1(v[decltype(K)::value]); });
     epilogue();
     }
+}
+
+template <int HLEN, int NV, int W, bool SPEC = false>
+__global__ __launch_bounds__(W == 1 ? 256 : 64 * W) void k_fwd2d_casc(const float* in, CascBands b, int Nr, int Nc, int VL,
+                                                                       float* __restrict__ trash, CascMap cm, TapsLH f)
+{
+    casc_fwd_body<HLEN, NV, W, SPEC, false>(in, b, Nr, Nc, VL, trash, cm, f);
+}
+template <int HLEN>
+__global__ __launch_bounds__(1024) void k_fwd2d_casc3f(const float* in, CascBands b, int Nr, int Nc, int VL, float* __restrict__ trash, CascMap cm,
+                                                       TapsLH f, CascL3 l3)
+{
+    (void)l3;
+    casc_fwd_body<HLEN, 2, 16, true, true>(in, b, Nr, Nc, VL, trash, cm, f);
 }
 
 template <int HLEN, int PFD>
@@ -751,8 +1028,60 @@
 
 static bool casc_enabled() { return knob(KN_CASC) == 1; }
 
+constexpr int kL3Tickets = 1 << 16;
+static std::mutex g_l3_mu;
+static unsigned* g_l3_tickets[64] = {};
+static bool g_l3_dirty[64] = {};
+static bool stream_is_capturing()
+{
+    hipStreamCaptureStatus st = hipStreamCaptureStatusNone;
+    if (hipStreamIsCapturing(stream(), &st) != hipSuccess) {
+        (void)hipGetLastError();
+        return true;
+    }
+    return st != hipStreamCaptureStatusNone;
+}
+static unsigned* l3_tickets()
+{
+    int dev = 0;
+    if (hipGetDevice(&dev) != hipSuccess || dev < 0 || dev >= 64 || user_stream_set()) return nullptr;
+    std::lock_guard<std::mutex> lk(g_l3_mu);
+    if (!g_l3_tickets[dev]) {
+        if (stream_is_capturing()) return nullptr;
+        void* p = nullptr;
+        if (hipMalloc(&p, (size_t)kL3Tickets * sizeof(unsigned)) != hipSuccess || hipMemset(p, 0, (size_t)kL3Tickets * sizeof(unsigned)) != hipSuccess) {
+            (void)hipGetLastError();
+            if (p) (void)hipFree(p);
+            return nullptr;
+        }
+        g_l3_tickets[dev] = (unsigned*)p;
+        g_l3_dirty[dev] = false;
+    }
+    if (g_l3_dirty[dev]) {
+        if (stream_is_capturing()) return nullptr;
+        if (hipMemsetAsync(g_l3_tickets[dev], 0, (size_t)kL3Tickets * sizeof(unsigned), stream()) != hipSuccess) {
+            (void)hipGetLastError();
+            return nullptr;
+        }
+        g_l3_dirty[dev] = false;
+    }
+    return g_l3_tickets[dev];
+}
+void casc_l3_prepare()
+{
+    if (knob(KN_CASC_L3F) == 1) (void)l3_tickets();
+}
+static void l3_tickets_failed()
+{
+    int dev = 0;
+    if (hipGetDevice(&dev) != hipSuccess || dev < 0 || dev >= 64) return;
+    std::lock_guard<std::mutex> lk(g_l3_mu);
+    g_l3_dirty[dev] = true;
+}
+
 template <int HLEN>
-static int launch_fwd_casc(const float* in, const CascBands& b, float* trash, int nr, int nc, const Taps2<float>& f2, const CascBatchF* d_tbl, int nimg)
+static int launch_fwd_casc(const float* in, const CascBands& b, float* trash, int nr, int nc, const Taps2<float>& f2, const CascBatchF* d_tbl, int nimg,
+                           CascL3Req* l3)
 {
     TapsLH f;
     for (int k = 0; k < PDWT_MAX_FILTER_WIDTH; k++) f.t[k] = v2f{f2.a[k], f2.b[k]};
@@ -810,6 +1139,31 @@
             }
             const CascMap cm = {idiv_up(nwg, 8), strips, gy, xw, d_tbl};
             const dim3 grid((unsigned)(8 * cm.cpx), (unsigned)(d_tbl ? nimg : 1));
+            if constexpr (HLEN == 4 || HLEN == 8) {
+                if (spec && xw == 0 && l3 && knob(KN_CASC_L3F) == 1 && !(nr & 7) && !(nc & 7) && gy >= 2 && strips >= 2 && (!d_tbl == !l3->tbl) &&
+                    (long long)nwg * (d_tbl ? nimg : 1) <= kL3Tickets) {
+                    int rmax = 0;
+                    bool ok = (nc / 4 - (strips - 1) * VL) >= HLEN && VL >= HLEN;
+                    for (int g = 0; g < gy && ok; g++) {
+                        const int R = casc_chunk_start(g + 1, 0, nr4, gy, strips, cm.cpx, 0) - casc_chunk_start(g, 0, nr4, gy, strips, cm.cpx, 0);
+                        ok = R >= HLEN;
+                        rmax = std::max(rmax, R);
+                    }
+                    const size_t lds3 = lds + 16 + std::max((size_t)rmax * 64 * sizeof(float), kL3BandBytes);
+                    unsigned* const tickets = (ok && rmax <= 99 && lds3 <= 160 * 1024) ? l3_tickets() : nullptr;
+                    if (tickets) {
+                        if (const int rc = lds_opt_in<k_fwd2d_casc3f<HLEN>>(); rc != PDWT_OK) return rc;
+                        const CascL3 a3 = {l3->A3, l3->H3, l3->V3, l3->D3, tickets, l3->tbl};
+                        PDWT_LAUNCH_KT(kt, k_fwd2d_casc3f<HLEN>, grid, dim3(64 * W), lds3, in, b, nr, nc, VL, trash, cm, f, a3);
+                        if (const hipError_t e = hipGetLastError(); e != hipSuccess) {
+                            l3_tickets_failed();
+                            PDWT_HIP_TRY(e);
+                        }
+                        l3->done = true;
+                        return PDWT_OK;
+                    }
+                }
+            }
             if (lds > 64 * 1024) {
                 int rc = (W == 4) ? lds_opt_in<k_fwd2d_casc<HLEN, NVD, 4>>()
                          : (W == 8) ? lds_opt_in<k_fwd2d_casc<HLEN, NVD, 8>>() : lds_opt_in<k_fwd2d_casc<HLEN, NVD, 16>>();
@@ -846,8 +1200,9 @@
 #endif
 
 int fwd2d_casc_f32(const float* in, float* H1, float* V1, float* D1, float* A2, float* H2, float* V2, float* D2, float* trash, int nr,
-                   int nc, int hlen, const Taps2<float>& f, const CascBatchF* d_tbl, int nimg)
-{
+                   int nc, int hlen, const Taps2<float>& f, const CascBatchF* d_tbl, int nimg, CascL3Req* l3)
+{
+    if (l3) l3->done = false;
     if (!casc_enabled() || !stream_enabled() || !trash) return 1;
     if ((nr & 3) || (nc & 3) || nc < 256 || nr < 16 * hlen) return 1;
     if ((long long)nr * nc < (long long)knob(KN_CASC_MIN)) return 1;
@@ -856,7 +1211,7 @@
     const CascBands b = {H1, V1, D1, A2, H2, V2, D2};
     switch (hlen) {
 #define X(H) \
-    case H: return launch_fwd_casc<H>(in, b, trash, nr, nc, f, d_tbl, nimg);
+    case H: return launch_fwd_casc<H>(in, b, trash, nr, nc, f, d_tbl, nimg, l3);
         PDWT_CASC_FWD_HLENS(X)
 #undef X
         default: return 1;
diff --git a/pdwt_amd/csrc/dwt_casc.hpp b/pdwt_amd/csrc/dwt_casc.hpp
--- a/pdwt_amd/csrc/dwt_casc.hpp
+++ b/pdwt_amd/csrc/dwt_casc.hpp
@@ -4,7 +4,7 @@
 
 namespace pdwt {
 int fwd2d_casc_f32(const float* in, float* H1, float* V1, float* D1, float* A2, float* H2, float* V2, float* D2, float* trash, int nr,
-                   int nc, int hlen, const Taps2<float>& f, const CascBatchF* d_tbl = nullptr, int nimg = 1);
+                   int nc, int hlen, const Taps2<float>& f, const CascBatchF* d_tbl = nullptr, int nimg = 1, CascL3Req* l3 = nullptr);
 int inv2d_casc_f32(const float* A2, const float* H2, const float* V2, const float* D2, const float* H1, const float* V1, const float* D1,
                    float* out, float* trash, int nr, int nc, int hlen, const Taps2<float>& f);
 }
diff --git a/pdwt_amd/csrc/runtime.hip b/pdwt_amd/csrc/runtime.hip
--- a/pdwt_amd/csrc/runtime.hip
+++ b/pdwt_amd/csrc/runtime.hip
@@ -37,6 +37,15 @@
         }
     }
     return g_streams[dev];
+}
+
+void casc_l3_prepare();
+bool user_stream_set()
+{
+    int dev = 0;
+    if (hipGetDevice(&dev) != hipSuccess || dev < 0 || dev >= 64) return true;
+    std::lock_guard<std::mutex> lk(g_mu);
+    return g_user_set[dev];
 }
 
 int lds_opt_in_ptr(const void* kernel)
@@ -68,6 +77,7 @@
     {"selfcheck", "PDWT_SELFCHECK", 1}, {"dwt1d_f64", "PDWT_DWT1D_F64", 1}, {"swtf_long", "PDWT_SWTF_LONG", 1}, {"f64_tail", "PDWT_F64_TAIL", 0},
     {"exp0", "PDWT_EXP0", 0}, {"exp1", "PDWT_EXP1", 0}, {"exp2", "PDWT_EXP2", 0}, {"exp3", "PDWT_EXP3", 0}, {"nonsep_tiled", "PDWT_NONSEP_TILED", 1},
     {"f64_lat", "PDWT_F64_LAT", 1}, {"f64_lat_min", "PDWT_F64_LAT_MIN", 4096}, {"dwt1d_nt_mb", "PDWT_DWT1D_NT_MB", 192},
+    {"casc_l3f", "PDWT_CASC_L3F", 1},
 };
 static int g_knob_vals[KN_COUNT];
 static std::once_flag g_knob_once;
@@ -324,6 +334,7 @@
 int pdwt_graph_capture_begin(void)
 {
     (void)pdwt::counted_waits_ok();
+    pdwt::casc_l3_prepare();
     PDWT_HIP_TRY(hipStreamBeginCapture(pdwt::stream(), hipStreamCaptureModeThreadLocal));
     return PDWT_OK;
 }
```

Result: slower. 263,200 Mpixels/s (-23.3%).
